# DichenZhang1/libultrahdr_dev

Hardware: AMD Instinct MI355X
Metric: MPixels/sec gain-map generate+apply, 4K P010 batch (higher is better)
Workload: dtype u8/u16 in, f32+f64 math, u8/u32 out

## Files before the change

libultrahdr_dev_amd/csrc/uhdr_capi.hip:

```cpp
#include <hip/hip_runtime.h>

#include <algorithm>
#include <memory>
#include <cmath>
#include <cstdio>
#include <cstring>
#include <map>
#include <chrono>
#include <mutex>
#include <thread>
#include <tuple>
#include <vector>

#include "../../include/uhdr_hip.h"
#include "uhdr_kernels.h"
#include "uhdr_jpeg.h"
#include "uhdr_jpegr.h"

namespace {

using namespace uhdr;

thread_local char t_err[256] = "";

void set_err(const char* where, hipError_t e) {
  snprintf(t_err, sizeof(t_err), "%s: %s", where, hipGetErrorString(e));
}

#define HIP_TRY(expr)                          \
  do {                                         \
    hipError_t _e = (expr);                    \
    if (_e != hipSuccess) {                    \
      set_err(#expr, _e);                      \
      return UHDR_HIP_UNKNOWN_ERROR;           \
    }                                          \
  } while (0)

constexpr int kStageSlots = 12;
struct StageSet {
  void* stage[kStageSlots] = {};
  size_t stage_bytes[kStageSlots] = {};
};
struct DeviceState : StageSet {
  bool ready = false;
  std::map<int, float*> idw;
  float* lut = nullptr;
  std::vector<std::unique_ptr<StageSet>> sets;
  std::vector<StageSet*> free_sets;
  std::vector<std::pair<hipStream_t, void*>> retired;
  std::vector<void*> pool;
  std::vector<size_t> pool_bytes;
  void* host_pool = nullptr;
  size_t host_pool_bytes = 0;
  std::map<hipStream_t, uint32_t*> stat_ws;
  struct ExWs { uint32_t* p = nullptr; size_t bytes = 0; };
  std::map<hipStream_t, ExWs> ex_ws;
  std::vector<std::unique_ptr<DeviceState>> codec_sets;
  std::vector<DeviceState*> free_codec;
};
std::mutex g_mu;
std::mutex g_pair_mu;
std::map<int, DeviceState> g_dev;

float euclid(float x1, float x2, float y1, float y2) {
  return (float)std::sqrt((double)(((y2 - y1) * (y2 - y1)) + (x2 - x1) * (x2 - x1)));
}
void fill_idw(float* w, int scale, int incR, int incB) {
  for (int y = 0; y < scale; y++)
    for (int x = 0; x < scale; x++) {
      const float pos_x = ((float)x) / scale, pos_y = ((float)y) / scale;
      const int curr_x = (int)std::floor((double)pos_x), curr_y = (int)std::floor((double)pos_y);
      const int next_x = curr_x + incR, next_y = curr_y + incB;
      const float d1 = euclid(pos_x, curr_x, pos_y, curr_y);
      float* o = w + y * scale * 4 + x * 4;
      if (d1 == 0) {
        o[0] = 1.f; o[1] = 0.f; o[2] = 0.f; o[3] = 0.f;
      } else {
        const float w1 = 1.f / d1;
        const float w2 = 1.f / euclid(pos_x, curr_x, pos_y, next_y);
        const float w3 = 1.f / euclid(pos_x, next_x, pos_y, curr_y);
        const float w4 = 1.f / euclid(pos_x, next_x, pos_y, next_y);
        const float total = w1 + w2 + w3 + w4;
        o[0] = w1 / total; o[1] = w2 / total; o[2] = w3 / total; o[3] = w4 / total;
      }
    }
}
void build_idw_tables(int scale, std::vector<float>& out) {
  const size_t n = (size_t)scale * scale * 4;
  out.assign(4 * n, 0.f);
  fill_idw(out.data(), scale, 1, 1);
  fill_idw(out.data() + n, scale, 0, 1);
  fill_idw(out.data() + 2 * n, scale, 1, 0);
  fill_idw(out.data() + 3 * n, scale, 0, 0);
}

int current_state(DeviceState** st) {
  int dev = -1;
  if (hipGetDevice(&dev) != hipSuccess) return UHDR_HIP_ERROR_INSUFFICIENT_RESOURCE;
  std::lock_guard<std::mutex> lk(g_mu);
  auto it = g_dev.find(dev);
  if (it == g_dev.end() || !it->second.ready) {
    snprintf(t_err, sizeof(t_err), "uhdr_hip_init(%d) has not been called", dev);
    return UHDR_HIP_ERROR_INSUFFICIENT_RESOURCE;
  }
  *st = &it->second;
  return UHDR_HIP_NO_ERROR;
}

constexpr int kIdwCacheMaxScale = 128;
int idw_for_scale(DeviceState* st, int scale, const float** dptr, float** transient) {
  *transient = nullptr;
  if (scale <= kIdwCacheMaxScale) {
    std::lock_guard<std::mutex> lk(g_mu);
    auto it = st->idw.find(scale);
    if (it != st->idw.end()) { *dptr = it->second; return UHDR_HIP_NO_ERROR; }
  }
  std::vector<float> t;
  try {
    build_idw_tables(scale, t);
  } catch (const std::bad_alloc&) {
    snprintf(t_err, sizeof(t_err), "no memory for the weight table of map scale %d", scale);
    return UHDR_HIP_ERROR_INSUFFICIENT_RESOURCE;
  }
  float* d = nullptr;
  if (hipMalloc(&d, t.size() * sizeof(float)) != hipSuccess) {
    (void)hipGetLastError();
    snprintf(t_err, sizeof(t_err), "no device memory for the weight table of map scale %d", scale);
    return UHDR_HIP_ERROR_INSUFFICIENT_RESOURCE;
  }
  if (hipMemcpy(d, t.data(), t.size() * sizeof(float), hipMemcpyHostToDevice) != hipSuccess) { (void)hipFree(d); return UHDR_HIP_UNKNOWN_ERROR; }
  if (scale > kIdwCacheMaxScale) { *transient = d; *dptr = d; return UHDR_HIP_NO_ERROR; }
  std::lock_guard<std::mutex> lk(g_mu);
  auto ins = st->idw.emplace(scale, d);
  if (!ins.second) (void)hipFree(d);
  *dptr = ins.first->second;
  return UHDR_HIP_NO_ERROR;
}

struct YuvRgb { float cr, gcb, gcr, cb; };
YuvRgb yuv_rgb_coeffs(int gamut) {
  switch (gamut) {
    case UHDR_HIP_CG_BT709: {
      const float R = 0.2126f, G = 0.7152f, B = 0.0722f, Cb = 1.8556f, Cr = 1.5748f;
      return {Cr, B * Cb / G, R * Cr / G, Cb};
    }
    case UHDR_HIP_CG_P3: {
      const float R = 0.299f, G = 0.587f, B = 0.114f, Cb = 1.772f, Cr = 1.402f;
      return {Cr, B * Cb / G, R * Cr / G, Cb};
    }
    default: {
      const float R = 0.2627f, G = 0.6780f, B = 0.0593f, Cb = 1.8814f, Cr = 1.4746f;
      return {Cr, B * Cb / G, R * Cr / G, Cb};
    }
  }
}
void luminance_coeffs(int gamut, float* o) {
  switch (gamut) {
    case UHDR_HIP_CG_BT709: o[0] = 0.2126f; o[1] = 0.7152f; o[2] = 0.0722f; break;
    case UHDR_HIP_CG_P3: o[0] = 0.20949f; o[1] = 0.72160f; o[2] = 0.06891f; break;
    default: o[0] = 0.2627f; o[1] = 0.6780f; o[2] = 0.0593f; break;
  }
}
const float kBt709ToP3[9] = {0.82254f, 0.17755f, 0.00006f, 0.03312f, 0.96684f, -0.00001f, 0.01706f, 0.07240f, 0.91049f};
const float kBt709ToBt2100[9] = {0.62740f, 0.32930f, 0.04332f, 0.06904f, 0.91958f, 0.01138f, 0.01636f, 0.08799f, 0.89555f};
const float kP3ToBt709[9] = {1.22482f, -0.22490f, -0.00007f, -0.04196f, 1.04199f, 0.00001f, -0.01961f, -0.07865f, 1.09831f};
const float kP3ToBt2100[9] = {0.75378f, 0.19862f, 0.04754f, 0.04576f, 0.94177f, 0.01250f, -0.00121f, 0.01757f, 0.98359f};
const float kBt2100ToBt709[9] = {1.66045f, -0.58764f, -0.07286f, -0.12445f, 1.13282f, -0.00837f, -0.01811f, -0.10057f, 1.11878f};
const float kBt2100ToP3[9] = {1.34369f, -0.28223f, -0.06135f, -0.06533f, 1.07580f, -0.01051f, 0.00283f, -0.01957f, 1.01679f};
const float* hdr_conversion(int sdr, int hdr) {
  if (sdr == hdr) return nullptr;
  switch (sdr) {
    case UHDR_HIP_CG_BT709: return hdr == UHDR_HIP_CG_P3 ? kP3ToBt709 : kBt2100ToBt709;
    case UHDR_HIP_CG_P3: return hdr == UHDR_HIP_CG_BT709 ? kBt709ToP3 : kBt2100ToP3;
    default: return hdr == UHDR_HIP_CG_BT709 ? kBt709ToBt2100 : kP3ToBt2100;
  }
}
const float kYuv709To601[9] = {1.0f, 0.101579f, 0.196076f, 0.0f, 0.989854f, -0.110653f, 0.0f, -0.072453f, 0.983398f};
const float kYuv709To2100[9] = {1.0f, -0.016969f, 0.096312f, 0.0f, 0.995306f, -0.051192f, 0.0f, 0.011507f, 1.002637f};
const float kYuv601To709[9] = {1.0f, -0.118188f, -0.212685f, 0.0f, 1.018640f, 0.114618f, 0.0f, 0.075049f, 1.025327f};
const float kYuv601To2100[9] = {1.0f, -0.128245f, -0.115879f, 0.0f, 1.010016f, 0.061592f, 0.0f, 0.086969f, 1.029350f};
const float kYuv2100To709[9] = {1.0f, 0.018149f, -0.095132f, 0.0f, 1.004123f, 0.051267f, 0.0f, -0.011524f, 0.996782f};
const float kYuv2100To601[9] = {1.0f, 0.117887f, 0.105521f, 0.0f, 0.995211f, -0.059549f, 0.0f, -0.084085f, 0.976518f};

bool valid_gamut(int g) { return g >= UHDR_HIP_CG_BT709 && g <= UHDR_HIP_CG_BT2100; }
bool al(const void* p, size_t a) { return (reinterpret_cast<uintptr_t>(p) % a) == 0; }

int validate_generate(const uhdr_hip_image_t* yuv, const uhdr_hip_image_t* p010, int hdr_tf,
                      const uhdr_hip_metadata_t* md, const uhdr_hip_image_t* dest) {
  if (yuv == nullptr || p010 == nullptr || md == nullptr || dest == nullptr || yuv->data == nullptr ||
      yuv->chroma_data == nullptr || p010->data == nullptr || p010->chroma_data == nullptr)
    return UHDR_HIP_ERROR_BAD_PTR;
  if (yuv->width != p010->width || yuv->height != p010->height) return UHDR_HIP_ERROR_RESOLUTION_MISMATCH;
  if (yuv->colorGamut == UHDR_HIP_CG_UNSPECIFIED || p010->colorGamut == UHDR_HIP_CG_UNSPECIFIED)
    return UHDR_HIP_ERROR_INVALID_COLORGAMUT;
  if (hdr_tf != UHDR_HIP_TF_LINEAR && hdr_tf != UHDR_HIP_TF_HLG && hdr_tf != UHDR_HIP_TF_PQ)
    return UHDR_HIP_ERROR_INVALID_TRANS_FUNC;
  if (!valid_gamut(yuv->colorGamut) || !valid_gamut(p010->colorGamut)) return UHDR_HIP_ERROR_INVALID_COLORGAMUT;
  return UHDR_HIP_NO_ERROR;
}

void fill_generate_metadata(int hdr_tf, uhdr_hip_metadata_t* md) {
  const float white = hdr_tf == UHDR_HIP_TF_PQ ? 10000.0f : 1000.0f;
  memset(md->version, 0, sizeof(md->version));
  strcpy(md->version, "1.0");
  md->maxContentBoost = white / 203.0f;
  md->minContentBoost = 1.0f;
  md->gamma = 1.0f;
  md->offsetSdr = 0.0f;
  md->offsetHdr = 0.0f;
  md->hdrCapacityMin = 1.0f;
  md->hdrCapacityMax = md->maxContentBoost;
}

void fill_generate_dest(const uhdr_hip_image_t* yuv, uhdr_hip_image_t* dest) {
  dest->width = yuv->width / 4;
  dest->height = yuv->height / 4;
  dest->colorGamut = UHDR_HIP_CG_UNSPECIFIED;
  dest->luma_stride = dest->width;
  dest->chroma_data = nullptr;
  dest->chroma_stride = 0;
  dest->pixelFormat = UHDR_HIP_PIX_FMT_MONOCHROME;
}

void encode_constants(float min_boost, float max_boost, float l2min, float l2max, double* scale, uint32_t* bmin,
                      uint32_t* bmax) {
  const double den = (double)(l2max - l2min);
  *scale = (double)255.0f / den;
  *bmin = (uint8_t)((std::log2((double)min_boost) - (double)l2min) / den * (double)255.0f);
  *bmax = (uint8_t)((std::log2((double)max_boost) - (double)l2min) / den * (double)255.0f);
}

GenConsts generate_consts(int sdr_gamut, int hdr_gamut, int hdr_tf, int sdr_is_601, size_t w, size_t h,
                          const uhdr_hip_metadata_t& md) {
  GenConsts c;
  const YuvRgb s = yuv_rgb_coeffs(sdr_is_601 ? UHDR_HIP_CG_P3 : sdr_gamut);
  const YuvRgb hh = yuv_rgb_coeffs(hdr_gamut);
  c.sdr_cr = s.cr; c.sdr_gcb = s.gcb; c.sdr_gcr = s.gcr; c.sdr_cb = s.cb;
  c.hdr_cr = hh.cr; c.hdr_gcb = hh.gcb; c.hdr_gcr = hh.gcr; c.hdr_cb = hh.cb;
  float l[3];
  luminance_coeffs(sdr_gamut, l);
  c.lum_r = l[0]; c.lum_g = l[1]; c.lum_b = l[2];
  const float* gm = hdr_conversion(sdr_gamut, hdr_gamut);
  c.gm_identity = gm == nullptr;
  for (int i = 0; i < 9; ++i) c.gm[i] = gm ? gm[i] : (i % 4 == 0 ? 1.0f : 0.0f);
  c.hdr_white_nits = hdr_tf == UHDR_HIP_TF_PQ ? 10000.0f : 1000.0f;
  c.min_boost = md.minContentBoost;
  c.max_boost = md.maxContentBoost;
  c.log2_min = (float)std::log2((double)md.minContentBoost);
  c.log2_max = (float)std::log2((double)md.maxContentBoost);
  encode_constants(c.min_boost, c.max_boost, c.log2_min, c.log2_max, &c.enc_scale, &c.enc_byte_min, &c.enc_byte_max);
  c.width = (uint32_t)w; c.height = (uint32_t)h;
  c.map_w = (uint32_t)(w / 4); c.map_h = (uint32_t)(h / 4);
  c.stat_keys = nullptr;
  c.stat_stride = 2;
  c.stat_ws = nullptr;
  c.stat_out = nullptr;
  c.stat_spread = 0u;
  c.stat_slots = 0u;
  c.lut = nullptr;
  c.bias4096 = 4096.0f;
  const double kRel = hdr_tf == UHDR_HIP_TF_PQ ? 1.0e-5 : 4.0e-6, kLogAbs = 5.0e-7;
  c.flt_scale = (float)c.enc_scale;
  c.flt_delta = (float)(1.25 * (c.enc_scale * (kRel * 1.4426950408889634 + kLogAbs) + 4.0e-5));
  c.flt_lo = (float)((double)c.min_boost * (1.0 - 2.0 * kRel));
  c.flt_hi = (float)((double)c.max_boost * (1.0 + 2.0 * kRel));
  c.flt_gain_rel = (float)(2.0 * kRel);
  return c;
}

GenImage gen_image(const uhdr_hip_image_t& yuv, const uhdr_hip_image_t& p010, void* map) {
  GenImage g;
  g.y = static_cast<const uint8_t*>(yuv.data);
  g.u = static_cast<const uint8_t*>(yuv.chroma_data);
  g.hy = static_cast<const uint16_t*>(p010.data);
  g.huv = static_cast<const uint16_t*>(p010.chroma_data);
  g.map = static_cast<uint8_t*>(map);
  g.y_stride = (uint32_t)yuv.luma_stride;
  g.c_stride = (uint32_t)yuv.chroma_stride;
  g.hy_stride = (uint32_t)(p010.luma_stride == 0 ? p010.width : p010.luma_stride);
  g.huv_stride = (uint32_t)p010.chroma_stride;
  return g;
}
bool gen_aligned(const GenImage& g, uint32_t w, uint32_t h) {
  const uint8_t* v = g.u + (size_t)g.c_stride * (h / 2u);
  if ((uint64_t)g.hy_stride * h >= (1ull << 31) || (uint64_t)g.y_stride * h >= (1ull << 32)) return false;
  return (w % 8u == 0) && al(g.hy, 16) && g.hy_stride % 8u == 0 && al(g.huv, 16) && g.huv_stride % 8u == 0 &&
         al(g.y, 8) && g.y_stride % 8u == 0 && al(g.u, 4) && al(v, 4) && g.c_stride % 4u == 0 && al(g.map, 2);
}

template <class F>
void chord(F f, double lo, double hi, double* c0, double* c1) {
  *c1 = (f(hi) - f(lo)) / (hi - lo);
  *c0 = f(lo) - *c1 * lo;
  double dev = 0.0;
  for (int k = 1; k < 32; ++k) { const double x = lo + (hi - lo) * k / 32.0; const double d = f(x) - (*c0 + *c1 * x); if (std::fabs(d) > std::fabs(dev)) dev = d; }
  *c0 += 0.5 * dev;
}
void f16_cell(uint32_t j, double* lo, double* hi) {
  const uint32_t e = j >> 7, m = j & 127u;
  if (e == 0) { *lo = std::ldexp((double)m, -21); *hi = std::ldexp((double)(m + 1u), -21); return; }
  *lo = std::ldexp(1.0 + m / 128.0, (int)e - 15);
  *hi = std::ldexp(1.0 + (m + 1u) / 128.0, (int)e - 15);
}
void f32_cell16(uint32_t j, double* lo, double* hi) {
  const uint32_t e = 96u + (j >> 4), m = j & 15u;
  *lo = std::ldexp(1.0 + m / 16.0, (int)e - 127);
  *hi = std::ldexp(1.0 + (m + 1u) / 16.0, (int)e - 127);
}
void build_stage1(double g, float* out) {
  const double thr = (double)0.04045f;
  auto eotf = [&](double x) { return x <= thr ? x / (double)12.92f : std::pow((x + (double)0.055f) / (double)1.055f, 2.4); };
  auto f = [&](double x) { return g == 1.0 ? eotf(x) : std::pow(eotf(x), g); };
  const uint32_t cells = (g == 1.0 ? kTabS1Bytes : kTabS1PowBytes) / 8u;
  for (uint32_t j = 0; j < cells; ++j) {
    double lo, hi, c0, c1;
    if (g == 1.0) f16_cell(j, &lo, &hi); else f32_cell16(j, &lo, &hi);
    if (g == 1.0 && hi <= thr) { c0 = 0.0; c1 = 1.0 / (double)12.92f; }
    else if (lo >= 1.0) { c0 = 1.0; c1 = 0.0; }
    else if (j == 0) { c0 = 0.0; c1 = f(hi) / hi; }
    else chord(f, lo, hi, &c0, &c1);
    out[2 * j] = (float)c0; out[2 * j + 1] = (float)c1;
  }
}
template <class F>
void build_stage2(F code_of_u, float* out) {
  for (uint32_t k = 0; k < kTabS2Cells; ++k) {
    const double lo = 2.0 + k / 64.0, hi = 2.0 + (k + 1u) / 64.0;
    auto f = [&](double s) { return code_of_u(std::min(1.0, 0.5 * (s - 2.0))); };
    float c0f = -2.0f, c1f = 0.0f;
    if (k == kTabS2Cells - 1u) c0f = (float)(-2.0 - std::ldexp(1023.0, -22));
    else if (f(hi) >= 0.99) {
      double c0, c1;
      chord(f, lo, hi, &c0, &c1);
      c0 += 1.0 / 256.0;
      const double n = c0 < 0.0 ? std::nearbyint(2.0 * c0) / 2.0 : std::nearbyint(c0);
      c1 += (c0 - n) / (0.5 * (lo + hi));
      c0f = (float)(-2.0 - std::ldexp(n, -22));
      c1f = (float)(-std::ldexp(c1, -22));
      auto at = [&](double s) { return -(((double)c1f * s + (double)c0f) + 2.0) * 4194304.0; };
      for (int it = 0; it < 4096 && at(lo) < 0.0; ++it) c1f = std::nextafter(c1f, -INFINITY);
      if (at(lo) < 0.0) { c0f = -2.0f; c1f = 0.0f; }
    }
    out[2 * k] = c0f; out[2 * k + 1] = c1f;
  }
}
void build_line_tables(std::vector<float>& tab) {
  tab.assign(kTabEnd - kTabS1Lin, 0.0f);
  const double m1 = (double)(2610.0f / 16384.0f), m2 = (double)(2523.0f / 4096.0f * 128.0f);
  const double k1 = (double)(3424.0f / 4096.0f), k2 = (double)(2413.0f / 4096.0f * 32.0f), k3 = (double)(2392.0f / 4096.0f * 32.0f);
  build_stage1(1.0, tab.data() + (kTabS1Lin - kTabS1Lin));
  build_stage1(0.5, tab.data() + (kTabS1Hlg - kTabS1Lin));
  build_stage1(m1, tab.data() + (kTabS1Pq - kTabS1Lin));
  auto hlg = [](double u) { const double x = u * u; return 1023.0 * (x <= 1.0 / 12.0 ? std::sqrt(3.0) * u : (double)0.17883277f * std::log(12.0 * x - (double)0.28466892f) + (double)0.55991073f); };
  auto pq = [&](double p) { return p <= 0.0 ? 0.0 : 1023.0 * std::pow((k1 + k2 * p) / (1.0 + k3 * p), m2); };
  build_stage2(hlg, tab.data() + (kTabS2Hlg - kTabS1Lin));
  build_stage2(pq, tab.data() + (kTabS2Pq - kTabS1Lin));
}

int validate_apply(const uhdr_hip_image_t* yuv, const uhdr_hip_image_t* map, const uhdr_hip_metadata_t* md,
                   const uhdr_hip_image_t* dest) {
  if (yuv == nullptr || map == nullptr || md == nullptr || dest == nullptr || yuv->data == nullptr ||
      yuv->chroma_data == nullptr || map->data == nullptr)
    return UHDR_HIP_ERROR_BAD_PTR;
  if (strncmp(md->version, "1.0", sizeof(md->version)) != 0) return UHDR_HIP_ERROR_BAD_METADATA;
  if (md->gamma != 1.0f) return UHDR_HIP_ERROR_BAD_METADATA;
  if (md->offsetSdr != 0.0f || md->offsetHdr != 0.0f) return UHDR_HIP_ERROR_BAD_METADATA;
  if (md->hdrCapacityMin != md->minContentBoost || md->hdrCapacityMax != md->maxContentBoost)
    return UHDR_HIP_ERROR_BAD_METADATA;
  if (map->width == 0 || map->height == 0) return UHDR_HIP_ERROR_UNSUPPORTED_MAP_SCALE_FACTOR;
  if (yuv->width % map->width != 0 || yuv->height % map->height != 0)
    return UHDR_HIP_ERROR_UNSUPPORTED_MAP_SCALE_FACTOR;
  if (yuv->width * map->height != yuv->height * map->width) return UHDR_HIP_ERROR_UNSUPPORTED_MAP_SCALE_FACTOR;
  return UHDR_HIP_NO_ERROR;
}
bool apply_writes(int fmt) {
  return fmt == UHDR_HIP_OUTPUT_HDR_LINEAR || fmt == UHDR_HIP_OUTPUT_HDR_PQ || fmt == UHDR_HIP_OUTPUT_HDR_HLG ||
         fmt == UHDR_HIP_OUTPUT_HDR_LINEAR_RGB_10BIT;
}
size_t apply_bpp(int fmt) {
  return fmt == UHDR_HIP_OUTPUT_HDR_LINEAR ? 8 : fmt == UHDR_HIP_OUTPUT_HDR_LINEAR_RGB_10BIT ? 6 : 4;
}
AppConsts apply_consts(const uhdr_hip_image_t& yuv, const uhdr_hip_image_t& map, const uhdr_hip_metadata_t& md,
                       float max_display_boost, const float* idw) {
  AppConsts c;
  c.width = (uint32_t)yuv.width; c.height = (uint32_t)yuv.height;
  c.map_w = (uint32_t)map.width; c.map_h = (uint32_t)map.height;
  c.scale = (uint32_t)(yuv.width / map.width);
  c.display_boost = (std::min)(max_display_boost, md.maxContentBoost);
  c.inv_display_boost = 1.0f / c.display_boost;
  c.max_boost = md.maxContentBoost;
  c.inv_max_boost = 1.0f / md.maxContentBoost;
  c.log2_min_d = std::log2((double)md.minContentBoost);
  c.log2_max_d = std::log2((double)md.maxContentBoost);
  c.idw = idw;
  c.lut = nullptr;
  c.lut_boost_factor = c.display_boost > 0 ? c.display_boost / md.maxContentBoost : 1.0f;
  const double lut_top = std::exp2(std::fmax(c.log2_min_d, c.log2_max_d) * (double)c.lut_boost_factor) / (double)c.display_boost;
  c.lut_plain_div = (c.display_boost >= 0x1p-20f && c.display_boost <= 0x1p20f && std::fabs(c.log2_min_d * (double)c.lut_boost_factor) <= 40.0 &&
                     std::fabs(c.log2_max_d * (double)c.lut_boost_factor) <= 40.0 && lut_top <= 32768.0) ? 1u : 0u;
  const double ratio = (double)c.display_boost / (double)md.maxContentBoost;
  c.fast.A = (float)((c.log2_max_d - c.log2_min_d) * ratio);
  c.fast.B = (float)(c.log2_min_d * ratio - std::log2((double)c.display_boost));
  c.fast.A255 = (float)((c.log2_max_d - c.log2_min_d) * ratio / 255.0);
  std::vector<float> t;
  build_idw_tables(4, t);
  for (int oy = 0; oy < 4; ++oy)
    for (int pr = 0; pr < 2; ++pr)
      for (int k = 1; k < 4; ++k)
        for (int j = 0; j < 2; ++j)
          c.fast.wD[oy][pr][k - 1][j] = t[oy * 16 + (2 * pr + j) * 4 + k];
  c.tab = nullptr;
  c.ex_ws = nullptr;
  c.ex_cap = 0;
  c.cells_per_thread = 8;
  c.step_x = c.step_y = 0;
  return c;
}
AppImage app_image(const uhdr_hip_image_t& yuv, const uhdr_hip_image_t& map, void* dst) {
  AppImage a;
  a.y = static_cast<const uint8_t*>(yuv.data);
  a.u = static_cast<const uint8_t*>(yuv.chroma_data);
  a.v = a.u + yuv.chroma_stride * (yuv.height / 2);
  a.map = static_cast<const uint8_t*>(map.data);
  a.dst = dst;
  a.y_stride = (uint32_t)yuv.luma_stride;
  a.c_stride = (uint32_t)yuv.chroma_stride;
  return a;
}
bool app_fast_s4(const AppConsts& c, const AppImage& a) {
  if ((uint64_t)a.y_stride * c.height >= (1ull << 32) || (uint64_t)c.width * c.height >= (1ull << 29)) return false;
  return c.scale == 4 && c.width == 4u * c.map_w && c.height == 4u * c.map_h && al(a.y, 4) && a.y_stride % 4u == 0 &&
         al(a.u, 2) && al(a.v, 2) && a.c_stride % 2u == 0 && al(a.dst, 16);
}
void fill_apply_dest(const uhdr_hip_image_t* yuv, uhdr_hip_image_t* dest) {
  dest->width = yuv->width;
  dest->height = yuv->height;
  dest->colorGamut = yuv->colorGamut;
}

int stage_reserve(StageSet* st, int slot, size_t bytes) {
  if (bytes == 0) bytes = 256;
  if (st->stage_bytes[slot] >= bytes) return UHDR_HIP_NO_ERROR;
  if (st->stage[slot]) HIP_TRY(hipFree(st->stage[slot]));
  st->stage[slot] = nullptr;
  st->stage_bytes[slot] = 0;
  HIP_TRY(hipMalloc(&st->stage[slot], bytes));
  st->stage_bytes[slot] = bytes;
  return UHDR_HIP_NO_ERROR;
}
size_t round_up(size_t v, size_t a) { return (v + a - 1) / a * a; }

class StageLease {
 public:
  explicit StageLease(DeviceState* st) : st_(st) {
    std::lock_guard<std::mutex> lk(g_mu);
    if (st_->free_sets.empty()) {
      try {
        st_->sets.emplace_back(new StageSet());
        set_ = st_->sets.back().get();
      } catch (const std::bad_alloc&) {
        set_ = nullptr;
      }
    } else {
      set_ = st_->free_sets.back();
      st_->free_sets.pop_back();
    }
  }
  ~StageLease() {
    if (set_ == nullptr) return;
    std::lock_guard<std::mutex> lk(g_mu);
    try { st_->free_sets.push_back(set_); } catch (const std::bad_alloc&) {}
  }
  StageLease(const StageLease&) = delete;
  StageLease& operator=(const StageLease&) = delete;
  StageSet* get() const { return set_; }
 private:
  DeviceState* st_;
  StageSet* set_;
};

class CodecLease {
 public:
  explicit CodecLease(DeviceState* st) : st_(st) {
    std::lock_guard<std::mutex> lk(g_mu);
    if (!st_->free_codec.empty()) {
      ctx_ = st_->free_codec.back();
      st_->free_codec.pop_back();
    } else {
      try {
        st_->free_codec.reserve(st_->codec_sets.size() + 1);
        st_->codec_sets.emplace_back(new DeviceState());
        ctx_ = st_->codec_sets.back().get();
      } catch (const std::bad_alloc&) {
        ctx_ = nullptr;
      }
    }
    if (ctx_) { ctx_->ready = true; ctx_->lut = st_->lut; }
  }
  ~CodecLease() {
    if (ctx_ == nullptr) return;
    std::lock_guard<std::mutex> lk(g_mu);
    st_->free_codec.push_back(ctx_);
  }
  CodecLease(const CodecLease&) = delete;
  CodecLease& operator=(const CodecLease&) = delete;
  DeviceState* get() const { return ctx_; }

 private:
  DeviceState* st_;
  DeviceState* ctx_ = nullptr;
};

int h2d_plane(void* d, size_t dpitch_elems, const void* h, size_t hstride_elems, size_t row_elems, size_t rows,
              size_t esz, hipStream_t s) {
  if (rows == 0 || row_elems == 0) return UHDR_HIP_NO_ERROR;
  if (hstride_elems == 0) {
    for (size_t r = 0; r < rows; ++r)
      HIP_TRY(hipMemcpyAsync(static_cast<char*>(d) + r * dpitch_elems * esz, h, row_elems * esz, hipMemcpyHostToDevice, s));
    return UHDR_HIP_NO_ERROR;
  }
  HIP_TRY(hipMemcpy2DAsync(d, dpitch_elems * esz, h, hstride_elems * esz, row_elems * esz, rows, hipMemcpyHostToDevice, s));
  return UHDR_HIP_NO_ERROR;
}
int d2h_plane(void* h, size_t hstride_elems, const void* d, size_t dpitch_elems, size_t row_elems, size_t rows,
              size_t esz, hipStream_t s) {
  if (rows == 0 || row_elems == 0) return UHDR_HIP_NO_ERROR;
  HIP_TRY(hipMemcpy2DAsync(h, hstride_elems * esz, d, dpitch_elems * esz, row_elems * esz, rows, hipMemcpyDeviceToHost, s));
  return UHDR_HIP_NO_ERROR;
}

int stage_yuv420_in(StageSet* st, int slot, const uhdr_hip_image_t& h, uhdr_hip_image_t* d, hipStream_t s) {
  const size_t w = h.width, hh = h.height, cw = (w + 1) / 2, ch = (hh + 1) / 2;
  const size_t lp = round_up(w ? w : 1, 64), cp = round_up(cw ? cw : 1, 64);
  int rc;
  if ((rc = stage_reserve(st, slot, lp * (hh ? hh : 1))) != 0) return rc;
  if ((rc = stage_reserve(st, slot + 1, cp * ((hh / 2) + ch + 1))) != 0) return rc;
  *d = h;
  d->data = st->stage[slot];
  d->chroma_data = st->stage[slot + 1];
  d->luma_stride = lp;
  d->chroma_stride = cp;
  if ((rc = h2d_plane(d->data, lp, h.data, h.luma_stride, w, hh, 1, s)) != 0) return rc;
  const uint8_t* hu = static_cast<const uint8_t*>(h.chroma_data);
  const uint8_t* hv = hu + h.chroma_stride * (hh / 2);
  uint8_t* du = static_cast<uint8_t*>(d->chroma_data);
  if ((rc = h2d_plane(du, cp, hu, h.chroma_stride, cw, ch, 1, s)) != 0) return rc;
  if ((rc = h2d_plane(du + cp * (hh / 2), cp, hv, h.chroma_stride, cw, ch, 1, s)) != 0) return rc;
  return UHDR_HIP_NO_ERROR;
}
int stage_p010_in(StageSet* st, int slot, const uhdr_hip_image_t& h, uhdr_hip_image_t* d, hipStream_t s) {
  const size_t w = h.width, hh = h.height, cw2 = ((w + 1) / 2) * 2, ch = (hh + 1) / 2;
  const size_t lp = round_up(w ? w : 1, 64), cp = round_up(cw2 ? cw2 : 2, 64);
  int rc;
  if ((rc = stage_reserve(st, slot, lp * (hh ? hh : 1) * 2)) != 0) return rc;
  if ((rc = stage_reserve(st, slot + 1, cp * (ch ? ch : 1) * 2)) != 0) return rc;
  *d = h;
  d->data = st->stage[slot];
  d->chroma_data = st->stage[slot + 1];
  d->luma_stride = lp;
  d->chroma_stride = cp;
  const size_t hls = h.luma_stride == 0 ? h.width : h.luma_stride;
// ... 1897 lines not shown
    memset(&e.sdr, 0, sizeof(e.sdr));
    if (api3) {
      const uint8_t* ip = nullptr;
      size_t in = 0;
      e.sdr_gamut = jpegr::first_icc(static_cast<const uint8_t*>(sdr_jpeg[i]), sdr_jpeg_size[i], &ip, &in) ? jpegr::gamut_from_icc(ip, in) : sdr_jpeg_gamut[i];
    } else {
      e.sdr = yuv420_images[i];
      default_yuv(&e.sdr);
      e.sdr_gamut = e.sdr.colorGamut;
      e.icc = std::move(icc[i]);
    }
    files.push_back(std::move(e));
  }
  auto result = [&]() {
    int first = UHDR_HIP_NO_ERROR;
    for (int i = 0; i < n; ++i) { if (status) status[i] = st_[i]; if (first == UHDR_HIP_NO_ERROR) first = st_[i]; }
    return first;
  };
  if (files.empty()) return result();
  DeviceState* st = nullptr;
  int rc = current_state(&st);
  size_t r0 = 0;
  if (rc == UHDR_HIP_NO_ERROR) {
    CodecLease lease(st);
    st = lease.get();
    rc = st == nullptr ? UHDR_HIP_ERROR_INSUFFICIENT_RESOURCE : UHDR_HIP_NO_ERROR;
    hipStream_t s = static_cast<hipStream_t>(stream);
    const bool host = mem_space != UHDR_HIP_MEM_DEVICE;
    auto key = [](const SjFile& e) { return std::make_tuple(e.p010.width, e.p010.height, e.sdr_gamut, e.p010.colorGamut); };
    std::stable_sort(files.begin(), files.end(), [&](const SjFile& x, const SjFile& y) { return key(x) < key(y); });
    struct SyncOnExit {
      hipStream_t s;
      ~SyncOnExit() { (void)hipStreamSynchronize(s); }
    } sync_on_exit{s};
    while (rc == UHDR_HIP_NO_ERROR && r0 < files.size()) {
      size_t r1 = r0, bytes = 0;
      while (r1 < files.size() && r1 - r0 < (size_t)kEncRound) {
        const size_t b = sj_round_bytes(files[r1], api3 ? &info[files[r1].idx] : nullptr, host);
        if (r1 > r0 && bytes + b > kCodecRoundBytes) break;
        bytes += b;
        ++r1;
      }
      rc = sdr_jpeg_round(st, s, api3, host, hdr_tf, &files[r0], (int)(r1 - r0), sdr_jpeg, sdr_jpeg_size, sdr_jpeg_gamut, api3 ? info.data() : nullptr,
                          dec_out.data(), dec_need.data(), out, out_capacity, out_size, st_.data());
      if (rc == UHDR_HIP_NO_ERROR) r0 = r1;
    }
  }
  for (size_t k = r0; k < files.size(); ++k)
    if (st_[files[k].idx] == UHDR_HIP_NO_ERROR) st_[files[k].idx] = rc;
  return result();
}

struct XFile {
  int idx = 0;
  uhdr_hip_image_t yuv, map;
  std::vector<uint8_t> icc;
};

int apix_round(DeviceState* st, hipStream_t s, bool host, int quality, const XFile* f, int m, const uhdr_hip_metadata_t* metadata,
               const void* const* exif, const size_t* exif_size, void* const* out, const size_t* out_capacity, size_t* out_size, int* st_) {
  std::vector<EncJpeg> jpg;
  jpg.reserve(2 * (size_t)m);
  int rc;
  if (host) {
    size_t total = 0;
    for (int k = 0; k < m; ++k) total += enc_stage_bytes(f[k].yuv) + enc_stage_bytes(f[k].map);
    if ((rc = pool_reserve(st, kEncYuv, total)) != 0) return rc;
  }
  size_t o = 0;
  for (int k = 0; k < m; ++k) {
    const XFile& e = f[k];
    jpg.push_back(EncJpeg{e.yuv, quality, &e.icc, e.yuv.luma_stride, e.yuv.chroma_stride});
    jpg.push_back(gainmap_jpeg(e.map, e.map.luma_stride));
    if (!host) continue;
    uint8_t* pool = static_cast<uint8_t*>(st->pool[kEncYuv]);
    if ((rc = stage_encoder_slice(pool + o, e.yuv, &jpg[2 * (size_t)k].img, s)) != 0) return rc;
    o += enc_stage_bytes(e.yuv);
    if ((rc = stage_encoder_slice(pool + o, e.map, &jpg[2 * (size_t)k + 1].img, s)) != 0) return rc;
    o += enc_stage_bytes(e.map);
  }
  if (compress_to_host(st, s, 2 * m, jpg.data()) != UHDR_HIP_NO_ERROR) return UHDR_HIP_ERROR_ENCODE_ERROR;
  on_host_threads(m, [&](int lo, int hi) {
    for (int k = lo; k < hi; ++k) {
      const int i = f[k].idx;
      const EncJpeg& sdr = jpg[2 * (size_t)k];
      const EncJpeg& gm = jpg[2 * (size_t)k + 1];
      st_[i] = jpegr::append_gainmap_to(sdr.bytes, sdr.n, gm.bytes, gm.n, static_cast<const uint8_t*>(exif ? exif[i] : nullptr), exif ? exif_size[i] : 0,
                                        nullptr, 0, metadata[i], static_cast<uint8_t*>(out[i]), out_capacity[i], &out_size[i]);
    }
  });
  return UHDR_HIP_NO_ERROR;
}
}

extern "C" {

int uhdr_hip_jpegr_encode_sdr_jpeg_batch(int n, const uhdr_hip_image_t* p010_images, const uhdr_hip_image_t* yuv420_images,
                                         const void* const* sdr_jpeg, const size_t* sdr_jpeg_size, const int* sdr_jpeg_gamut, int hdr_tf,
                                         void* const* out, const size_t* out_capacity, size_t* out_size, int* status, int mem_space, void* stream) {
  if (n < 0 || (n > 0 && (p010_images == nullptr || sdr_jpeg == nullptr || sdr_jpeg_size == nullptr || sdr_jpeg_gamut == nullptr || out == nullptr ||
                          out_capacity == nullptr || out_size == nullptr)))
    return UHDR_HIP_ERROR_BAD_PTR;
  return sdr_jpeg_files(n, p010_images, yuv420_images, sdr_jpeg, sdr_jpeg_size, sdr_jpeg_gamut, hdr_tf, out, out_capacity, out_size, status,
                        mem_space, stream);
}

int uhdr_hip_jpegr_encode_apix_batch(int n, const uhdr_hip_image_t* yuv420_images, const uhdr_hip_image_t* gainmap_images,
                                     const uhdr_hip_metadata_t* metadata, int quality, const void* const* exif, const size_t* exif_size,
                                     void* const* out, const size_t* out_capacity, size_t* out_size, int* status, int mem_space, void* stream) {
  if (n < 0 || (n > 0 && (yuv420_images == nullptr || gainmap_images == nullptr || metadata == nullptr || out == nullptr || out_capacity == nullptr ||
                          out_size == nullptr)) ||
      (exif != nullptr && exif_size == nullptr))
    return UHDR_HIP_ERROR_BAD_PTR;
  if (quality < 0 || quality > 100) return UHDR_HIP_ERROR_INVALID_QUALITY_FACTOR;
  std::vector<int> st_((size_t)n, UHDR_HIP_NO_ERROR);
  std::vector<XFile> files;
  for (int i = 0; i < n; ++i) {
    const uhdr_hip_image_t& y = yuv420_images[i];
    const uhdr_hip_image_t& g = gainmap_images[i];
    if (y.data == nullptr || g.data == nullptr || out[i] == nullptr) { st_[i] = UHDR_HIP_ERROR_BAD_PTR; continue; }
    XFile e;
    e.idx = i;
    int rc = apix_check(y, g, &e.yuv, &e.map, &e.icc);
    if (rc == UHDR_HIP_NO_ERROR && !jpegr::metadata_valid(metadata[i])) rc = UHDR_HIP_ERROR_BAD_METADATA;
    if (rc != UHDR_HIP_NO_ERROR) { st_[i] = rc; continue; }
    files.push_back(std::move(e));
  }
  auto result = [&]() {
    int first = UHDR_HIP_NO_ERROR;
    for (int i = 0; i < n; ++i) { if (status) status[i] = st_[i]; if (first == UHDR_HIP_NO_ERROR) first = st_[i]; }
    return first;
  };
  if (files.empty()) return result();
  DeviceState* st = nullptr;
  int rc = current_state(&st);
  size_t r0 = 0;
  if (rc == UHDR_HIP_NO_ERROR) {
    CodecLease lease(st);
    st = lease.get();
    rc = st == nullptr ? UHDR_HIP_ERROR_INSUFFICIENT_RESOURCE : UHDR_HIP_NO_ERROR;
    hipStream_t s = static_cast<hipStream_t>(stream);
    const bool host = mem_space != UHDR_HIP_MEM_DEVICE;
    struct SyncOnExit {
      hipStream_t s;
      ~SyncOnExit() { (void)hipStreamSynchronize(s); }
    } sync_on_exit{s};
    while (rc == UHDR_HIP_NO_ERROR && r0 < files.size()) {
      size_t r1 = r0, bytes = 0;
      while (r1 < files.size() && r1 - r0 < (size_t)kEncRound) {
        const size_t b = enc_round_bytes(files[r1].yuv, host, true) + enc_round_bytes(files[r1].map, host, true);
        if (r1 > r0 && bytes + b > kCodecRoundBytes) break;
        bytes += b;
        ++r1;
      }
      rc = apix_round(st, s, host, quality, &files[r0], (int)(r1 - r0), metadata, exif, exif_size, out, out_capacity, out_size, st_.data());
      if (rc == UHDR_HIP_NO_ERROR) r0 = r1;
    }
  }
  for (size_t k = r0; k < files.size(); ++k) st_[files[k].idx] = rc;
  return result();
}

int uhdr_hip_jpegr_info(const void* jpegr, size_t jpegr_size, uhdr_hip_jpeg_info_t* primary, uhdr_hip_jpeg_info_t* gainmap) {
  if (jpegr == nullptr || primary == nullptr) return UHDR_HIP_ERROR_BAD_PTR;
  const uint8_t* file = static_cast<const uint8_t*>(jpegr);
  jpegr::Range img[2];
  const int found = jpegr::find_images(file, jpegr_size, img);
  if (found == 0) return UHDR_HIP_ERROR_NO_IMAGES_FOUND;
  if (found == 1) return UHDR_HIP_ERROR_GAIN_MAP_IMAGE_NOT_FOUND;
  auto parse = [&](const jpegr::Range& r, uhdr_hip_jpeg_info_t* info) -> int {
    const uint8_t* j = file + r.begin;
    struct { int w, h; } di;
    if (!jpegr::has_valid_header(j, r.len) || !jpegr::dimensions(j, r.len, &di.w, &di.h)) return UHDR_HIP_ERROR_DECODE_ERROR;
    if (di.w > 8192 || di.h > 8192) return UHDR_HIP_ERROR_DECODE_ERROR;
    memset(info, 0, sizeof(*info));
    info->offset = r.begin; info->size = r.len;
    info->width = (size_t)di.w; info->height = (size_t)di.h;
    jpegr::first_packets(j, r.len, &info->xmp_offset, &info->xmp_size, &info->exif_offset, &info->exif_size, &info->icc_offset, &info->icc_size);
    if (info->xmp_size) info->xmp_offset += r.begin;
    if (info->exif_size) info->exif_offset += r.begin;
    if (info->icc_size) info->icc_offset += r.begin;
    return UHDR_HIP_NO_ERROR;
  };
  int rc = parse(img[0], primary);
  if (rc != UHDR_HIP_NO_ERROR) return rc;
  return gainmap != nullptr ? parse(img[1], gainmap) : UHDR_HIP_NO_ERROR;
}

int uhdr_hip_jpegr_metadata(const void* jpegr, size_t jpegr_size, uhdr_hip_metadata_t* metadata) {
  if (jpegr == nullptr || metadata == nullptr) return UHDR_HIP_ERROR_BAD_PTR;
  const uint8_t* file = static_cast<const uint8_t*>(jpegr);
  jpegr::Range img[2];
  const int found = jpegr::find_images(file, jpegr_size, img);
  if (found == 0) return UHDR_HIP_ERROR_NO_IMAGES_FOUND;
  if (found == 1) return UHDR_HIP_ERROR_GAIN_MAP_IMAGE_NOT_FOUND;
  const uint8_t* xmp = nullptr;
  size_t xmp_len = 0;
  if (!jpegr::first_xmp(file + img[1].begin, img[1].len, &xmp, &xmp_len) ||
      !jpegr::metadata_from_xmp(xmp, xmp_len, metadata))
    return UHDR_HIP_ERROR_METADATA_ERROR;
  return UHDR_HIP_NO_ERROR;
}

int uhdr_hip_lut_table(int which, float* out, size_t capacity, size_t* count) {
  if (out == nullptr || count == nullptr) return UHDR_HIP_ERROR_BAD_PTR;
  DeviceState* st = nullptr;
  const int rc = current_state(&st);
  if (rc != UHDR_HIP_NO_ERROR) return rc;
  uint32_t off = 0, n = 0;
  switch (which) {
    case 0: off = kLutSrgbInv; n = kLutSrgbInvN; break;
    case 1: off = kLutHlgInv; n = kLutHlgInvN; break;
    case 2: off = kLutPqInv; n = kLutPqInvN; break;
    case 4: off = kLutHlg; n = kLutHlgN; break;
    case 5: off = kLutPq; n = kLutPqN; break;
    default: return UHDR_HIP_ERROR_UNSUPPORTED_FEATURE;
  }
  *count = n;
  if (capacity < n) return UHDR_HIP_ERROR_INSUFFICIENT_RESOURCE;
  HIP_TRY(hipMemcpy(out, st->lut + off, sizeof(float) * n, hipMemcpyDeviceToHost));
  return UHDR_HIP_NO_ERROR;
}

int uhdr_hip_gain_lut(const uhdr_hip_metadata_t* metadata, int with_display_boost, float display_boost, float* out) {
  if (metadata == nullptr || out == nullptr) return UHDR_HIP_ERROR_BAD_PTR;
  DeviceState* st = nullptr;
  int rc = current_state(&st);
  if (rc != UHDR_HIP_NO_ERROR) return rc;
  float factor = 1.0f;
  if (with_display_boost) factor = display_boost > 0 ? display_boost / metadata->maxContentBoost : 1.0f;
  CodecLease lease(st);
  if ((st = lease.get()) == nullptr) return UHDR_HIP_ERROR_INSUFFICIENT_RESOURCE;
  if ((rc = stage_reserve(st, 6, sizeof(float) * kGainLutN)) != 0) return rc;
  float* d = static_cast<float*>(st->stage[6]);
  HIP_TRY(launch_build_gain_lut(d, std::log2((double)metadata->minContentBoost), std::log2((double)metadata->maxContentBoost),
                                factor, nullptr));
  HIP_TRY(hipMemcpy(out, d, sizeof(float) * kGainLutN, hipMemcpyDeviceToHost));
  return UHDR_HIP_NO_ERROR;
}

int uhdr_hip_idw_tables(int scale, float* out) {
  if (out == nullptr || scale <= 0) return UHDR_HIP_ERROR_BAD_PTR;
  std::vector<float> t;
  build_idw_tables(scale, t);
  memcpy(out, t.data(), t.size() * sizeof(float));
  return UHDR_HIP_NO_ERROR;
}

int uhdr_hip_generate_gainmap_batch(int n, const uhdr_hip_image_t* yuvs, const uhdr_hip_image_t* p010s, int hdr_tf,
                                    uhdr_hip_metadata_t* metadata, uhdr_hip_image_t* dests, int sdr_is_601,
                                    float* content_minmax, void* stream) {
  return uhdr_hip_generate_gainmap_batch_ex(n, yuvs, p010s, hdr_tf, metadata, dests, sdr_is_601, UHDR_HIP_GENERATE_EXACT,
                                            content_minmax, stream);
}

int uhdr_hip_generate_gainmap_batch_ex(int n, const uhdr_hip_image_t* yuvs, const uhdr_hip_image_t* p010s, int hdr_tf,
                                       uhdr_hip_metadata_t* metadata, uhdr_hip_image_t* dests, int sdr_is_601,
                                       int generate_mode, float* content_minmax, void* stream) {
  if (generate_mode != UHDR_HIP_GENERATE_EXACT && generate_mode != UHDR_HIP_GENERATE_LUT &&
      generate_mode != UHDR_HIP_GENERATE_UNFILTERED)
    return UHDR_HIP_ERROR_UNSUPPORTED_FEATURE;
  const bool lut = generate_mode == UHDR_HIP_GENERATE_LUT;
  if (n < 0 || (n > 0 && (yuvs == nullptr || p010s == nullptr || dests == nullptr)) || metadata == nullptr)
    return UHDR_HIP_ERROR_BAD_PTR;
  for (int i = 0; i < n; ++i) {
    const int rc = validate_generate(&yuvs[i], &p010s[i], hdr_tf, metadata, &dests[i]);
    if (rc != UHDR_HIP_NO_ERROR) return rc;
    if (dests[i].data == nullptr) return UHDR_HIP_ERROR_BAD_PTR;
  }
  if (hdr_tf != UHDR_HIP_TF_LINEAR && hdr_tf != UHDR_HIP_TF_HLG && hdr_tf != UHDR_HIP_TF_PQ)
    return UHDR_HIP_ERROR_INVALID_TRANS_FUNC;
  DeviceState* st = nullptr;
  int rc = current_state(&st);
  if (rc != UHDR_HIP_NO_ERROR) return rc;
  hipStream_t s = static_cast<hipStream_t>(stream);

  fill_generate_metadata(hdr_tf, metadata);
  uint32_t* keys = reinterpret_cast<uint32_t*>(content_minmax);

  int i = 0;
  while (i < n) {
    const uhdr_hip_image_t& y0 = yuvs[i];
    GenConsts c = generate_consts(y0.colorGamut, p010s[i].colorGamut, hdr_tf, sdr_is_601, y0.width, y0.height, *metadata);
    c.stat_keys = keys ? keys + 2 * i : nullptr;
    c.stat_stride = 2;
    c.lut = lut ? st->lut : nullptr;
    GenBatch b;
    int m = 0;
    bool aligned = true;
    while (i + m < n && m < kMaxChunk) {
      const uhdr_hip_image_t& y = yuvs[i + m];
      if (y.width != y0.width || y.height != y0.height || y.colorGamut != y0.colorGamut ||
          p010s[i + m].colorGamut != p010s[i].colorGamut)
        break;
      b.img[m] = gen_image(y, p010s[i + m], dests[i + m].data);
      const bool a = gen_aligned(b.img[m], c.width, c.height);
      if (m == 0) aligned = a;
      else if (a != aligned) break;
      fill_generate_dest(&y, &dests[i + m]);
      ++m;
    }
    bool filter = generate_mode == UHDR_HIP_GENERATE_EXACT && c.flt_delta < 0.25f && c.min_boost >= 0.25f && c.max_boost <= 64.0f;
    const bool small = generate_is_small(c, m);
    const bool pair = keys != nullptr ? generate_resolve_pays(c, m) : !small;
    if (keys != nullptr && !pair) filter = false;
    const bool resolve = filter && aligned && !lut && pair;
    std::unique_lock<std::mutex> pair_lk(g_pair_mu, std::defer_lock);
    if (resolve) pair_lk.lock();
    if (resolve) {
      uint32_t* w = nullptr;
      const int wrc = stat_workspace(st, s, &w);
      if (wrc != UHDR_HIP_NO_ERROR) return wrc;
      c.stat_ws = w;
      c.stat_keys = keys ? w + 4 : nullptr;
      c.stat_stride = kStatWords;
      c.stat_out = keys ? content_minmax + 2 * i : nullptr;
      c.stat_spread = (m <= 16 && (uint64_t)((c.map_w + 1u) >> 1) * c.map_h >= 512u * 64u) ? 1u : 0u;
      c.stat_slots = generate_slot_waves(c, m);
    } else if (keys != nullptr) {
      HIP_TRY(launch_stats_init(keys + 2 * i, m, s));
    }
    HIP_TRY(launch_generate(c, b, m, hdr_tf, aligned, lut, filter, s));
    if (resolve) HIP_TRY(launch_stats_resolve(c, b, m, hdr_tf, aligned, s));
    else if (keys != nullptr) HIP_TRY(launch_stats_finalize(keys + 2 * i, m, s));
    i += m;
  }
  return UHDR_HIP_NO_ERROR;
}

int uhdr_hip_apply_gainmap_batch(int n, const uhdr_hip_image_t* yuvs, const uhdr_hip_image_t* maps,
                                 const uhdr_hip_metadata_t* metadata, int output_format, float max_display_boost,
                                 uhdr_hip_image_t* dests, int apply_mode, void* stream) {
  if (n < 0 || (n > 0 && (yuvs == nullptr || maps == nullptr || dests == nullptr)) || metadata == nullptr)
    return UHDR_HIP_ERROR_BAD_PTR;
  for (int i = 0; i < n; ++i) {
    const int rc = validate_apply(&yuvs[i], &maps[i], metadata, &dests[i]);
    if (rc != UHDR_HIP_NO_ERROR) return rc;
  }
  if (apply_mode != UHDR_HIP_APPLY_FAST && apply_mode != UHDR_HIP_APPLY_EXACT && apply_mode != UHDR_HIP_APPLY_LUT &&
      apply_mode != UHDR_HIP_APPLY_EXACT_UNFILTERED)
    return UHDR_HIP_ERROR_UNSUPPORTED_FEATURE;
  DeviceState* st = nullptr;
  int rc = current_state(&st);
  if (rc != UHDR_HIP_NO_ERROR) return rc;
  hipStream_t s = static_cast<hipStream_t>(stream);
  const bool writes = apply_writes(output_format);
  for (int i = 0; i < n; ++i)
    if (writes && dests[i].data == nullptr) return UHDR_HIP_ERROR_BAD_PTR;

  int i = 0;
  while (i < n) {
    const uhdr_hip_image_t& y0 = yuvs[i];
    const uhdr_hip_image_t& m0 = maps[i];
    const int scale = (int)(y0.width / m0.width);
    const float* idw = nullptr;
    float* idw_transient = nullptr;
    if ((rc = idw_for_scale(st, scale, &idw, &idw_transient)) != UHDR_HIP_NO_ERROR) return rc;
    struct FreeAfter {
      float* p; hipStream_t s;
      ~FreeAfter() { if (p) { (void)hipStreamSynchronize(s); (void)hipFree(p); } }
    } free_after{idw_transient, s};
    AppConsts c = apply_consts(y0, m0, *metadata, max_display_boost, idw);
    c.lut = apply_mode == UHDR_HIP_APPLY_LUT ? st->lut : nullptr;
    c.tab = st->lut;
    AppBatch b;
    int m = 0;
    bool fast = true;
    while (i + m < n && m < kMaxChunk) {
      const uhdr_hip_image_t& y = yuvs[i + m];
      const uhdr_hip_image_t& mp = maps[i + m];
      if (y.width != y0.width || y.height != y0.height || mp.width != m0.width || mp.height != m0.height) break;
      b.img[m] = app_image(y, mp, dests[i + m].data);
      const bool f = app_fast_s4(c, b.img[m]);
      if (m == 0) fast = f;
      else if (f != fast) break;
      fill_apply_dest(&y, &dests[i + m]);
      ++m;
    }
    std::unique_lock<std::mutex> pair_lk(g_pair_mu, std::defer_lock);
    if (writes && apply_mode == UHDR_HIP_APPLY_EXACT && (uint64_t)c.width * c.height <= 0xFFFFFFFFull &&
        std::fabs(c.log2_min_d) <= 32.0 && std::fabs(c.log2_max_d) <= 32.0) {
      pair_lk.lock();
      const uint32_t cap = ex_list_cap((uint64_t)c.width * c.height);
      uint32_t* w = nullptr;
      const int wrc = exact_workspace(st, s, m, cap, &w);
      if (wrc != UHDR_HIP_NO_ERROR) return wrc;
      c.ex_ws = w;
      c.ex_cap = cap;
    }
    if (writes) HIP_TRY(launch_apply(c, b, m, output_format, apply_mode, fast, s));
    i += m;
  }
  return UHDR_HIP_NO_ERROR;
}

int uhdr_hip_generate_gainmap(const uhdr_hip_image_t* yuv, const uhdr_hip_image_t* p010, int hdr_tf,
                              uhdr_hip_metadata_t* metadata, uhdr_hip_image_t* dest, int sdr_is_601, int mem_space,
                              void* stream) {
  return uhdr_hip_generate_gainmap_ex(yuv, p010, hdr_tf, metadata, dest, sdr_is_601, UHDR_HIP_GENERATE_EXACT, mem_space, stream);
}

int uhdr_hip_generate_gainmap_ex(const uhdr_hip_image_t* yuv, const uhdr_hip_image_t* p010, int hdr_tf,
                                 uhdr_hip_metadata_t* metadata, uhdr_hip_image_t* dest, int sdr_is_601, int generate_mode,
                                 int mem_space, void* stream) {
  int rc = validate_generate(yuv, p010, hdr_tf, metadata, dest);
  if (rc != UHDR_HIP_NO_ERROR) return rc;
  if (dest->data == nullptr) return UHDR_HIP_ERROR_BAD_PTR;
  if (mem_space == UHDR_HIP_MEM_DEVICE)
    return uhdr_hip_generate_gainmap_batch_ex(1, yuv, p010, hdr_tf, metadata, dest, sdr_is_601, generate_mode, nullptr, stream);

  DeviceState* st = nullptr;
  if ((rc = current_state(&st)) != UHDR_HIP_NO_ERROR) return rc;
  StageLease lease(st);
  StageSet* ss = lease.get();
  if (ss == nullptr) return UHDR_HIP_ERROR_INSUFFICIENT_RESOURCE;
  hipStream_t s = static_cast<hipStream_t>(stream);
  uhdr_hip_image_t dy, dp, dm = *dest;
  if ((rc = stage_yuv420_in(ss, 0, *yuv, &dy, s)) != 0) return rc;
  if ((rc = stage_p010_in(ss, 2, *p010, &dp, s)) != 0) return rc;
  const size_t mw = yuv->width / 4, mh = yuv->height / 4;
  if ((rc = stage_reserve(ss, 4, mw * mh)) != 0) return rc;
  dm.data = ss->stage[4];
  rc = uhdr_hip_generate_gainmap_batch_ex(1, &dy, &dp, hdr_tf, metadata, &dm, sdr_is_601, generate_mode, nullptr, stream);
  if (rc != UHDR_HIP_NO_ERROR) return rc;
  if (mw * mh) HIP_TRY(hipMemcpyAsync(dest->data, dm.data, mw * mh, hipMemcpyDeviceToHost, s));
  HIP_TRY(hipStreamSynchronize(s));
  fill_generate_dest(yuv, dest);
  return UHDR_HIP_NO_ERROR;
}

int uhdr_hip_apply_gainmap(const uhdr_hip_image_t* yuv, const uhdr_hip_image_t* map, const uhdr_hip_metadata_t* metadata,
                           int output_format, float max_display_boost, uhdr_hip_image_t* dest, int apply_mode,
                           int mem_space, void* stream) {
  int rc = validate_apply(yuv, map, metadata, dest);
  if (rc != UHDR_HIP_NO_ERROR) return rc;
  if (mem_space == UHDR_HIP_MEM_DEVICE)
    return uhdr_hip_apply_gainmap_batch(1, yuv, map, metadata, output_format, max_display_boost, dest, apply_mode, stream);

  const bool writes = apply_writes(output_format);
  if (writes && dest->data == nullptr) return UHDR_HIP_ERROR_BAD_PTR;
  DeviceState* st = nullptr;
  if ((rc = current_state(&st)) != UHDR_HIP_NO_ERROR) return rc;
  StageLease lease(st);
  StageSet* ss = lease.get();
  if (ss == nullptr) return UHDR_HIP_ERROR_INSUFFICIENT_RESOURCE;
  hipStream_t s = static_cast<hipStream_t>(stream);
  uhdr_hip_image_t dy, dm = *map, dd = *dest;
  if ((rc = stage_yuv420_in(ss, 0, *yuv, &dy, s)) != 0) return rc;
  const size_t map_bytes = map->width * map->height;
  if ((rc = stage_reserve(ss, 4, map_bytes)) != 0) return rc;
  HIP_TRY(hipMemcpyAsync(ss->stage[4], map->data, map_bytes, hipMemcpyHostToDevice, s));
  dm.data = ss->stage[4];
  const size_t out_bytes = writes ? yuv->width * yuv->height * apply_bpp(output_format) : 0;
  if ((rc = stage_reserve(ss, 5, out_bytes)) != 0) return rc;
  dd.data = ss->stage[5];
  rc = uhdr_hip_apply_gainmap_batch(1, &dy, &dm, metadata, output_format, max_display_boost, &dd, apply_mode, stream);
  if (rc != UHDR_HIP_NO_ERROR) return rc;
  if (out_bytes) HIP_TRY(hipMemcpyAsync(dest->data, dd.data, out_bytes, hipMemcpyDeviceToHost, s));
  HIP_TRY(hipStreamSynchronize(s));
  fill_apply_dest(yuv, dest);
  return UHDR_HIP_NO_ERROR;
}

namespace {
ToneImage tone_image(const uhdr_hip_image_t& sd, const uhdr_hip_image_t& dd, bool* aligned) {
  ToneImage t;
  t.sy = static_cast<const uint16_t*>(sd.data);
  t.suv = static_cast<const uint16_t*>(sd.chroma_data);
  t.dy = static_cast<uint8_t*>(dd.data);
  t.du = static_cast<uint8_t*>(dd.chroma_data);
  t.dv = t.du + (dd.chroma_stride * dd.height / 2);
  t.sy_stride = (uint32_t)sd.luma_stride; t.suv_stride = (uint32_t)sd.chroma_stride;
  t.dy_stride = (uint32_t)dd.luma_stride; t.dc_stride = (uint32_t)dd.chroma_stride;
  t.width = (uint32_t)sd.width; t.height = (uint32_t)sd.height;
  *aligned = t.width % 16u == 0 && al(t.sy, 16) && t.sy_stride % 8u == 0 && al(t.suv, 16) &&
             t.suv_stride % 8u == 0 && al(t.dy, 8) && t.dy_stride % 8u == 0 && t.dy_stride >= t.width &&
             al(t.du, 8) && al(t.dv, 8) && t.dc_stride % 8u == 0 && t.dc_stride >= t.width / 2u;
  return t;
}
int tonemap_check(const uhdr_hip_image_t* src, const uhdr_hip_image_t* dest) {
  if (src == nullptr || dest == nullptr) return UHDR_HIP_ERROR_BAD_PTR;
  if (src->width != dest->width || src->height != dest->height) return UHDR_HIP_ERROR_RESOLUTION_MISMATCH;
  if (src->data == nullptr || src->chroma_data == nullptr || dest->data == nullptr || dest->chroma_data == nullptr)
    return UHDR_HIP_ERROR_BAD_PTR;
  return UHDR_HIP_NO_ERROR;
}
}

int uhdr_hip_tonemap_batch(int n, const uhdr_hip_image_t* srcs, uhdr_hip_image_t* dests, void* stream) {
  if (n < 0 || (n > 0 && (srcs == nullptr || dests == nullptr))) return UHDR_HIP_ERROR_BAD_PTR;
  for (int i = 0; i < n; ++i) {
    const int rc = tonemap_check(&srcs[i], &dests[i]);
    if (rc != UHDR_HIP_NO_ERROR) return rc;
  }
  DeviceState* st = nullptr;
  int rc = current_state(&st);
  if (rc != UHDR_HIP_NO_ERROR) return rc;
  hipStream_t s = static_cast<hipStream_t>(stream);
  int i = 0;
  while (i < n) {
    ToneBatch b;
    bool aligned = true;
    int m = 0;
    while (i + m < n && m < kToneChunk) {
      bool a;
      const ToneImage t = tone_image(srcs[i + m], dests[i + m], &a);
      if (m == 0) aligned = a;
      else if (a != aligned || t.width != b.img[0].width || t.height != b.img[0].height) break;
      b.img[m++] = t;
    }
    HIP_TRY(launch_tonemap(b, m, aligned, s));
    for (int k = 0; k < m; ++k) dests[i + k].colorGamut = srcs[i + k].colorGamut;
    i += m;
  }
  return UHDR_HIP_NO_ERROR;
}

int uhdr_hip_tonemap(const uhdr_hip_image_t* src, uhdr_hip_image_t* dest, int mem_space, void* stream) {
  int rc = tonemap_check(src, dest);
  if (rc != UHDR_HIP_NO_ERROR) return rc;
  if (mem_space == UHDR_HIP_MEM_DEVICE) return uhdr_hip_tonemap_batch(1, src, dest, stream);
  DeviceState* st = nullptr;
  if ((rc = current_state(&st)) != UHDR_HIP_NO_ERROR) return rc;
  hipStream_t s = static_cast<hipStream_t>(stream);

  auto run = [&](const uhdr_hip_image_t& sd, const uhdr_hip_image_t& dd) -> int {
    ToneBatch b;
    bool aligned;
    b.img[0] = tone_image(sd, dd, &aligned);
    HIP_TRY(launch_tonemap(b, 1, aligned, s));
    return UHDR_HIP_NO_ERROR;
  };

  StageLease lease(st);
  StageSet* ss = lease.get();
  if (ss == nullptr) return UHDR_HIP_ERROR_INSUFFICIENT_RESOURCE;
  uhdr_hip_image_t ds, dd = *dest;
  if ((rc = stage_p010_in(ss, 2, *src, &ds, s)) != 0) return rc;
  const size_t h = dest->height, ls = dest->luma_stride, cs = dest->chroma_stride;
  if ((rc = stage_reserve(ss, 0, ls * h)) != 0) return rc;
  if ((rc = stage_reserve(ss, 1, cs * h + cs)) != 0) return rc;
  dd.data = ss->stage[0];
  dd.chroma_data = ss->stage[1];
  if ((rc = run(ds, dd)) != 0) return rc;
  if (ls * h) HIP_TRY(hipMemcpyAsync(dest->data, dd.data, ls * h, hipMemcpyDeviceToHost, s));
  const size_t v_off = cs * h / 2;
  if (cs * (h / 2)) {
    HIP_TRY(hipMemcpyAsync(dest->chroma_data, dd.chroma_data, cs * (h / 2), hipMemcpyDeviceToHost, s));
    HIP_TRY(hipMemcpyAsync(static_cast<uint8_t*>(dest->chroma_data) + v_off, static_cast<uint8_t*>(dd.chroma_data) + v_off,
                           cs * (h / 2), hipMemcpyDeviceToHost, s));
  }
  HIP_TRY(hipStreamSynchronize(s));
  dest->colorGamut = src->colorGamut;
  return UHDR_HIP_NO_ERROR;
}

namespace {
int convert_check(const uhdr_hip_image_t* image, int src_encoding, int dest_encoding) {
  if (image == nullptr) return UHDR_HIP_ERROR_BAD_PTR;
  if (src_encoding == UHDR_HIP_CG_UNSPECIFIED || dest_encoding == UHDR_HIP_CG_UNSPECIFIED)
    return UHDR_HIP_ERROR_INVALID_COLORGAMUT;
  if (!valid_gamut(src_encoding) || !valid_gamut(dest_encoding)) return UHDR_HIP_ERROR_INVALID_COLORGAMUT;
  return UHDR_HIP_NO_ERROR;
}
}

int uhdr_hip_convert_yuv_batch(int n, uhdr_hip_image_t* images, int src_encoding, int dest_encoding, void* stream) {
  if (n < 0 || (n > 0 && images == nullptr)) return UHDR_HIP_ERROR_BAD_PTR;
  int rc = convert_check(n > 0 ? &images[0] : nullptr, src_encoding, dest_encoding);
  if (n == 0) rc = (src_encoding == UHDR_HIP_CG_UNSPECIFIED || dest_encoding == UHDR_HIP_CG_UNSPECIFIED || !valid_gamut(src_encoding) ||
                    !valid_gamut(dest_encoding)) ? UHDR_HIP_ERROR_INVALID_COLORGAMUT : UHDR_HIP_NO_ERROR;
  if (rc != UHDR_HIP_NO_ERROR) return rc;
  if (src_encoding == dest_encoding) return UHDR_HIP_NO_ERROR;
  for (int i = 0; i < n; ++i)
    if (images[i].data == nullptr || images[i].chroma_data == nullptr) return UHDR_HIP_ERROR_BAD_PTR;
  const float* m = yuv_matrix(src_encoding, dest_encoding);
  DeviceState* st = nullptr;
  if ((rc = current_state(&st)) != UHDR_HIP_NO_ERROR) return rc;
  hipStream_t s = static_cast<hipStream_t>(stream);
  int i = 0;
  while (i < n) {
    CvtBatch b;
    bool aligned = true;
    int k = 0;
    while (i + k < n && k < kToneChunk) {
      bool a;
      const CvtImage t = cvt_image(images[i + k], images[i + k], m, &a);
      if (k == 0) aligned = a;
      else if (a != aligned || t.width != b.img[0].width || t.height != b.img[0].height) break;
      b.img[k++] = t;
    }
    HIP_TRY(launch_convert_yuv(b, k, aligned, s));
    i += k;
  }
  return UHDR_HIP_NO_ERROR;
}

int uhdr_hip_convert_yuv(uhdr_hip_image_t* image, int src_encoding, int dest_encoding, int mem_space, void* stream) {
  int rc = convert_check(image, src_encoding, dest_encoding);
  if (rc != UHDR_HIP_NO_ERROR) return rc;
  if (src_encoding == dest_encoding) return UHDR_HIP_NO_ERROR;
  if (image->data == nullptr || image->chroma_data == nullptr) return UHDR_HIP_ERROR_BAD_PTR;
  if (mem_space == UHDR_HIP_MEM_DEVICE) return uhdr_hip_convert_yuv_batch(1, image, src_encoding, dest_encoding, stream);
  const float* m = yuv_matrix(src_encoding, dest_encoding);
  DeviceState* st = nullptr;
  if ((rc = current_state(&st)) != UHDR_HIP_NO_ERROR) return rc;
  hipStream_t s = static_cast<hipStream_t>(stream);
  auto run = [&](const uhdr_hip_image_t& d) -> int { return convert_yuv_into(d, d, m, s); };
  StageLease lease(st);
  if (lease.get() == nullptr) return UHDR_HIP_ERROR_INSUFFICIENT_RESOURCE;
  uhdr_hip_image_t d;
  if ((rc = stage_yuv420_in(lease.get(), 0, *image, &d, s)) != 0) return rc;
  if ((rc = run(d)) != 0) return rc;
  const size_t w = image->width, h = image->height, cw = w / 2, ch = h / 2;
  if ((rc = d2h_plane(image->data, image->luma_stride, d.data, d.luma_stride, cw * 2, ch * 2, 1, s)) != 0) return rc;
  uint8_t* hu = static_cast<uint8_t*>(image->chroma_data);
  const uint8_t* du = static_cast<const uint8_t*>(d.chroma_data);
  if ((rc = d2h_plane(hu, image->chroma_stride, du, d.chroma_stride, cw, ch, 1, s)) != 0) return rc;
  if ((rc = d2h_plane(hu + image->chroma_stride * (h / 2), image->chroma_stride, du + d.chroma_stride * (h / 2),
                      d.chroma_stride, cw, ch, 1, s)) != 0)
    return rc;
  HIP_TRY(hipStreamSynchronize(s));
  return UHDR_HIP_NO_ERROR;
}

namespace {
enum { FXK_CROP, FXK_MIRROR, FXK_ROTATE, FXK_RESIZE };
// ... 227 lines not shown
```

libultrahdr_dev_amd/csrc/uhdr_kernels.h:

```cpp
#pragma once
#include <hip/hip_runtime_api.h>
#include <stdint.h>

namespace uhdr {

constexpr uint32_t kStatSlotWaves = 1024, kStatSlotPlain = 15, kStatSlotSaved = 4, kStatSlotWords = 16 + 16 * kStatSlotSaved;
constexpr uint32_t kStatLists = 64, kStatCap = 252, kStatEst = 8 + kStatLists, kStatSlotCnt = kStatEst + 2 * kStatLists,
                   kStatHdr = kStatSlotCnt + kStatSlotWaves,
                   kStatWords = kStatHdr + (kStatLists * kStatCap > kStatSlotWaves * kStatSlotWords ? kStatLists * kStatCap : kStatSlotWaves * kStatSlotWords);
static_assert(kStatHdr % 4u == 0u && kStatSlotWords % 4u == 0u && kStatWords % 4u == 0u, "saved entries are read and written as 16-byte pieces");
constexpr int kMaxChunk = 64;

constexpr uint32_t kLutSrgbInvN = 1024, kLutHlgInvN = 4096, kLutPqInvN = 4096, kLutHlgN = 65536, kLutPqN = 65536;
constexpr uint32_t kLutSrgbInv = 0, kLutHlgInv = kLutSrgbInv + kLutSrgbInvN, kLutPqInv = kLutHlgInv + kLutHlgInvN,
                   kLutHlg = kLutPqInv + kLutPqInvN, kLutPq = kLutHlg + kLutHlgN, kLutTotal = kLutPq + kLutPqN;
constexpr uint32_t kTabS1Bytes = 0x3C00 + 16;
constexpr uint32_t kTabS1PowBytes = 512u * 8u;
constexpr uint32_t kTabS2Cells = 129, kTabS2Floats = 260;
constexpr uint32_t kTabS2LdsBytes = kTabS2Cells * 256u;
constexpr uint32_t kTabS1Lin = kLutTotal, kTabS1Hlg = kTabS1Lin + kTabS1Bytes / 4, kTabS1Pq = kTabS1Hlg + kTabS1PowBytes / 4,
                   kTabS2Hlg = kTabS1Pq + kTabS1PowBytes / 4, kTabS2Pq = kTabS2Hlg + kTabS2Floats, kTabEnd = kTabS2Pq + kTabS2Floats;
constexpr uint32_t kCodeHlg = kTabEnd, kCodePq = kCodeHlg + kLutHlgN / 2, kLutBufferFloats = kCodePq + kLutPqN / 2;
constexpr uint32_t kGainLutN = 1024;

struct GenConsts {
  float sdr_cr, sdr_gcb, sdr_gcr, sdr_cb;
  float hdr_cr, hdr_gcb, hdr_gcr, hdr_cb;
  float lum_r, lum_g, lum_b;
  float gm[9];
  int gm_identity;
  float hdr_white_nits;
  float bias4096;
  float min_boost, max_boost, log2_min, log2_max;
  double enc_scale;
  uint32_t enc_byte_min, enc_byte_max;
  uint32_t width, height, map_w, map_h;
  uint32_t* stat_keys;
  uint32_t stat_stride;
  uint32_t* stat_ws;
  float* stat_out;
  const float* lut;
  float flt_scale, flt_delta, flt_lo, flt_hi;
  float flt_gain_rel;
  uint32_t stat_spread;
  uint32_t stat_slots;
};
struct EvalConsts {
  float min_boost, max_boost, log2_min, log2_max;
  double enc_scale;
  uint32_t enc_byte_min, enc_byte_max;
  const float* lut;
  double log2_min_d, log2_max_d;
};
struct GenImage {
  const uint8_t* y;
  const uint8_t* u;
  const uint16_t* hy;
  const uint16_t* huv;
  uint8_t* map;
  uint32_t y_stride, c_stride, hy_stride, huv_stride;
};
struct GenBatch {
  GenImage img[kMaxChunk];
};

struct AppFast {
  float A, B, A255;
  float wD[4][2][3][2];
};
struct AppConsts {
  uint32_t width, height, map_w, map_h, scale;
  uint32_t cells_per_thread;
  uint32_t step_x, step_y;
  float display_boost, inv_display_boost, max_boost, inv_max_boost;
  double log2_min_d, log2_max_d;
  const float* idw;
  const float* lut;
  const float* tab;
  float lut_boost_factor;
  uint32_t lut_plain_div;
  uint32_t* ex_ws;
  uint32_t ex_cap;
  AppFast fast;
};
constexpr uint32_t kExLists = 1024;
constexpr uint32_t kExHdrWords = 8 + kExLists;
inline size_t ex_ws_bytes(uint32_t cap) { return ((size_t)kMaxChunk * kExHdrWords + (size_t)kMaxChunk * kExLists * cap) * 4u; }
inline uint32_t ex_list_cap(uint64_t pixels) { return (uint32_t)(pixels / 16u / kExLists) + 64u; }
struct AppImage {
  const uint8_t* y;
  const uint8_t* u;
  const uint8_t* v;
  const uint8_t* map;
  void* dst;
  uint32_t y_stride, c_stride;
};
struct AppBatch {
  AppImage img[kMaxChunk];
};

struct ToneImage {
  const uint16_t* sy;
  const uint16_t* suv;
  uint8_t* dy;
  uint8_t* du;
  uint8_t* dv;
  uint32_t sy_stride, suv_stride, dy_stride, dc_stride;
  uint32_t width, height;
};
constexpr int kToneChunk = 32;
struct ToneBatch {
  ToneImage img[kToneChunk];
};
struct CvtImage {
  uint8_t* y;
  uint8_t* u;
  uint8_t* v;
  uint32_t y_stride, c_stride, width, height;
  float m[9];
  const uint8_t* sy;
  const uint8_t* su;
  const uint8_t* sv;
  uint32_t sy_stride, sc_stride;
};
struct CvtBatch {
  CvtImage img[kToneChunk];
};

enum FxOp : int { FX_COPY = 0, FX_FLIP_V, FX_FLIP_H, FX_ROT90, FX_ROT180, FX_ROT270, FX_RESIZE };
struct FxJob {
  const uint8_t* src;
  uint8_t* dst;
  uint32_t rows, cols, dst_stride, src_stride;
  uint32_t in_w, in_h;
  uint32_t row_num, row_den, col_num, col_den;
  int op;
};
struct FxJobs {
  FxJob job[3];
  int n;
};

static_assert(sizeof(GenConsts) + sizeof(GenBatch) <= 4096, "generate kernel arguments exceed the kernarg segment");
static_assert(sizeof(AppConsts) + sizeof(AppBatch) <= 4096, "apply kernel arguments exceed the kernarg segment");

hipError_t launch_generate(const GenConsts& c, const GenBatch& b, int n, int hdr_tf, bool aligned, bool lut,
                           bool filter, hipStream_t s);
bool generate_is_small(const GenConsts& c, int n);
bool generate_resolve_pays(const GenConsts& c, int n);
uint32_t generate_slot_waves(const GenConsts& c, int n);
hipError_t launch_stats_init(uint32_t* keys, int n, hipStream_t s);
hipError_t launch_stats_resolve(const GenConsts& c, const GenBatch& b, int n, int hdr_tf, bool aligned, hipStream_t s);
constexpr size_t kStatWsBytes = sizeof(uint32_t) * kStatWords * (size_t)kMaxChunk;
hipError_t launch_stats_finalize(uint32_t* keys, int n, hipStream_t s);
hipError_t launch_apply(const AppConsts& c, const AppBatch& b, int n, int fmt, int mode,
                        bool fast_s4, hipStream_t s);
hipError_t launch_build_luts(float* lut , hipStream_t s);
hipError_t launch_build_lut_codes(float* lut , hipStream_t s);
hipError_t launch_build_gain_lut(float* table, double log2_min, double log2_max, float boost_factor, hipStream_t s);
hipError_t launch_tonemap(const ToneBatch& b, int n, bool aligned, hipStream_t s);
hipError_t launch_convert_yuv(const CvtBatch& b, int n, bool aligned, hipStream_t s);
static_assert(sizeof(CvtBatch) <= 4096 && sizeof(ToneBatch) <= 4096, "toneMap / convertYuv kernel arguments exceed the kernarg segment");
hipError_t launch_ycc420_to_rgba(const uint8_t* y, const uint8_t* cb, const uint8_t* cr, uint32_t w, uint32_t h, uint32_t y_stride,
                                 uint32_t c_stride, uint8_t* rgba, hipStream_t s);
constexpr int kRgbaChunk = 64;
struct YccRgbaImage {
  const uint8_t* y;
  const uint8_t* cb;
  const uint8_t* cr;
  uint8_t* rgba;
  uint32_t w, h, ys, cs;
};
struct YccRgbaBatch {
  YccRgbaImage img[kRgbaChunk];
};
static_assert(sizeof(YccRgbaBatch) <= 4096, "k_ycc420_rgba_batch's kernel arguments exceed the kernarg segment");
hipError_t launch_ycc420_to_rgba_batch(const YccRgbaBatch& b, int n, hipStream_t s);
hipError_t upload_idw4(const float* tables );
hipError_t launch_effect(const FxJobs& j, hipStream_t s);
hipError_t launch_eval_transfer(int fn, const float* in, float* out, size_t n, const EvalConsts& ec, hipStream_t s);
hipError_t launch_synth_lcg(uint16_t* p010, uint8_t* yuv, uint32_t n_luma, uint32_t n, uint32_t seed, hipStream_t s);

}
```

libultrahdr_dev_amd/csrc/uhdr_kernels.hip:

```cpp
#include "uhdr_kernels.h"

#include <hip/hip_runtime.h>

#include <algorithm>
#include <cmath>

#include "uhdr_device_math.h"
#include "uhdr_wave_scan.h"

namespace uhdr {

__constant__ float c_idw4[4 * 64];

__constant__ float c_idw4p[64];

hipError_t upload_idw4(const float* tables) {
  float p[64];
  for (int oy = 0; oy < 4; ++oy)
    for (int pr = 0; pr < 2; ++pr)
      for (int k = 0; k < 4; ++k)
        for (int h = 0; h < 2; ++h) p[((oy * 2 + pr) * 4 + k) * 2 + h] = tables[oy * 16 + (2 * pr + h) * 4 + k];
  hipError_t e = hipMemcpyToSymbol(HIP_SYMBOL(c_idw4p), p, sizeof(p));
  if (e != hipSuccess) return e;
  return hipMemcpyToSymbol(HIP_SYMBOL(c_idw4), tables, sizeof(float) * 4 * 64);
}

constexpr float k255 = 1 / 255.0f;
constexpr float k876 = 1 / 876.0f;
constexpr float k896 = 1 / 896.0f;

constexpr float kP3YR = 0.299f, kP3YG = 0.587f, kP3YB = 0.114f;
constexpr float kP3Cb = 1.772f, kP3Cr = 1.402f;
constexpr float kP3GCb = kP3YB * kP3Cb / kP3YG;
constexpr float kP3GCr = kP3YR * kP3Cr / kP3YG;

typedef float f2 __attribute__((ext_vector_type(2)));
__device__ __forceinline__ f2 pk_fma(f2 a, f2 b, f2 c) { return __builtin_elementwise_fma(a, b, c); }
__device__ __forceinline__ f2 splat(float v) { return (f2){v, v}; }
__device__ __forceinline__ f2 bc_lo(f2 v) { return __builtin_shufflevector(v, v, 0, 0); }
__device__ __forceinline__ f2 bc_hi(f2 v) { return __builtin_shufflevector(v, v, 1, 1); }

__device__ __forceinline__ f2 pk_add_sat(f2 a, f2 b) {
  f2 r;
  asm("v_pk_add_f32 %0, %1, %2 clamp" : "=v"(r) : "v"(a), "v"(b));
  return r;
}
__device__ __forceinline__ f2 pk_mul_sat(f2 a, f2 b) {
  f2 r;
  asm("v_pk_mul_f32 %0, %1, %2 clamp" : "=v"(r) : "v"(a), "v"(b));
  return r;
}
__device__ __forceinline__ f2 pk_fma_sat(f2 a, f2 b, f2 c) {
  f2 r;
  asm("v_pk_fma_f32 %0, %1, %2, %3 clamp" : "=v"(r) : "v"(a), "v"(b), "v"(c));
  return r;
}

template <int HI>
__device__ __forceinline__ f2 pk_fma_sat_bc(f2 a, f2 b, f2 c) {
  f2 r;
  if (HI) asm("v_pk_fma_f32 %0, %1, %2, %3 op_sel:[0,0,1] op_sel_hi:[1,1,1] clamp" : "=v"(r) : "v"(a), "v"(b), "v"(c));
  else asm("v_pk_fma_f32 %0, %1, %2, %3 op_sel_hi:[1,1,0] clamp" : "=v"(r) : "v"(a), "v"(b), "v"(c));
  return r;
}


__device__ __attribute__((noinline)) uint32_t lut_index_wild(float t) {
  const double pos = (double)t + 0.5;
  uint32_t v = 0u;
  if (__builtin_fabs(pos) < 9223372036854775808.0) v = (uint32_t)(long long)pos;
  return v;
}
__device__ __forceinline__ uint32_t round_half_up(float t) {
  int r;
  asm("v_cvt_rpi_i32_f32 %0, %1" : "=v"(r) : "v"(t));
  return (uint32_t)r;
}
__device__ __forceinline__ uint32_t lut_index(float e, uint32_t n) {
  const float t = e * (float)(n - 1u);
  uint32_t v;
  if (__builtin_expect(__float_as_uint(t) < 0x4F000000u, 1)) v = round_half_up(t);
  else v = lut_index_wild(t);
  return min(v, n - 1u);
}
__device__ __forceinline__ uint32_t lut_index_unit(float e, uint32_t n) {
  return round_half_up(e * (float)(n - 1u));
}
__device__ __forceinline__ float gain_lut_entry(uint32_t idx, double log2_min, double log2_max, float boost_factor) {
  const float value = (float)idx / (float)(kGainLutN - 1u);
  const float log_boost = (float)(log2_min * (double)(1.0f - value) + log2_max * (double)value);
  return (float)exp2((double)(log_boost * boost_factor));
}

__global__ void __launch_bounds__(256) k_build_luts(float* lut) {
  const uint32_t i = blockIdx.x * 256u + threadIdx.x;
  if (i >= kLutTotal) return;
  float y;
  if (i < kLutHlgInv) y = srgb_inv_oetf_exact((float)(i - kLutSrgbInv) / (float)(kLutSrgbInvN - 1u));
  else if (i < kLutPqInv) y = hlg_inv_oetf_exact((float)(i - kLutHlgInv) / (float)(kLutHlgInvN - 1u));
  else if (i < kLutHlg) y = pq_inv_oetf_exact((float)(i - kLutPqInv) / (float)(kLutPqInvN - 1u));
  else if (i < kLutPq) y = hlg_oetf_exact((float)(i - kLutHlg) / (float)(kLutHlgN - 1u));
  else y = pq_oetf_exact((float)(i - kLutPq) / (float)(kLutPqN - 1u));
  lut[i] = y;
}
hipError_t launch_build_luts(float* lut, hipStream_t s) {
  hipLaunchKernelGGL(k_build_luts, dim3((kLutTotal + 255u) / 256u), dim3(256), 0, s, lut);
  return hipGetLastError();
}
__global__ void __launch_bounds__(256) k_build_lut_codes(float* lut) {
  const uint32_t i = blockIdx.x * 256u + threadIdx.x;
  const uint32_t t = i >> 16, k = i & 0xFFFFu;
  uint16_t* codes = reinterpret_cast<uint16_t*>(lut + (t ? kCodePq : kCodeHlg));
  codes[k] = (uint16_t)(0x3ffu & (uint32_t)(lut[(t ? kLutPq : kLutHlg) + k] * 1023.0f));
}
hipError_t launch_build_lut_codes(float* lut, hipStream_t s) {
  hipLaunchKernelGGL(k_build_lut_codes, dim3(2u * 65536u / 256u), dim3(256), 0, s, lut);
  return hipGetLastError();
}
__global__ void __launch_bounds__(256) k_build_gain_lut(float* table, double log2_min, double log2_max, float boost_factor) {
  const uint32_t i = blockIdx.x * 256u + threadIdx.x;
  if (i < kGainLutN) table[i] = gain_lut_entry(i, log2_min, log2_max, boost_factor);
}
hipError_t launch_build_gain_lut(float* table, double log2_min, double log2_max, float boost_factor, hipStream_t s) {
  hipLaunchKernelGGL(k_build_gain_lut, dim3(kGainLutN / 256u), dim3(256), 0, s, table, log2_min, log2_max, boost_factor);
  return hipGetLastError();
}


template <int TF>
__device__ __forceinline__ float hdr_inv_oetf(float e) {
  if (TF == 1) return hlg_inv_oetf_guarded(e);
  if (TF == 2) return pq_inv_oetf_guarded(e);
  return e;
}

__device__ __forceinline__ float cvt_word0(uint32_t w) {
  float r;
  asm("v_cvt_f32_u32_sdwa %0, %1 dst_sel:DWORD dst_unused:UNUSED_PAD src0_sel:WORD_0" : "=v"(r) : "v"(w));
  return r;
}
__device__ __forceinline__ float cvt_word1(uint32_t w) {
  float r;
  asm("v_cvt_f32_u32_sdwa %0, %1 dst_sel:DWORD dst_unused:UNUSED_PAD src0_sel:WORD_1" : "=v"(r) : "v"(w));
  return r;
}


constexpr int kGenWhole = 0, kGenFront = 1, kGenBack = 2;
struct GenMid { f2 r, g, b, hr, hg, hb; };
template <int TF, bool LUT, bool FILTER, bool DEFER = false, int PART = kGenWhole>
__device__ __forceinline__ uint32_t gen_pair(const GenConsts& c, const uint32_t (&hy)[2][4][2],
                                             const uint32_t (&huv)[2][2][2], const uint32_t (&y8)[2][4],
                                             const uint32_t (&u8)[2][2], const uint32_t (&v8)[2][2],
                                             uint8_t (&out)[2], float (&gain)[2], const float* s_srgb, const float* s_hdr,
                                             GenMid* mid = nullptr) {
  f2 r, g, b, hr, hg, hb;
  if (PART == kGenBack) {
    r = mid->r; g = mid->g; b = mid->b; hr = mid->hr; hg = mid->hg; hb = mid->hb;
  } else {
  f2 sy = splat(0.0f), su = splat(0.0f), sv = splat(0.0f);
  f2 hsy = splat(0.0f), hsu = splat(0.0f), hsv = splat(0.0f);
#pragma unroll
  for (int r = 0; r < 2; ++r) {
    f2 uf[2], vf[2], huf[2], hvf[2];
#pragma unroll
    for (int k = 0; k < 2; ++k) {
      const f2 ub = (f2){(float)((u8[0][r] >> (8 * k)) & 0xffu), (float)((u8[1][r] >> (8 * k)) & 0xffu)};
      const f2 vb = (f2){(float)((v8[0][r] >> (8 * k)) & 0xffu), (float)((v8[1][r] >> (8 * k)) & 0xffu)};
      uf[k] = pk_fma(ub, splat(k255), splat(-128.0f * k255));
      vf[k] = pk_fma(vb, splat(k255), splat(-128.0f * k255));
      const uint32_t m0 = huv[0][r][k] & 0xFFC0FFC0u, m1 = huv[1][r][k] & 0xFFC0FFC0u;
      const f2 hu = (f2){cvt_word0(m0), cvt_word0(m1)};
      const f2 hv = (f2){cvt_word1(m0), cvt_word1(m1)};
      huf[k] = pk_fma(hu, splat(k896 * 0.015625f), splat(-64.0f * k896)) - splat(0.5f);
      hvf[k] = pk_fma(hv, splat(k896 * 0.015625f), splat(-64.0f * k896)) - splat(0.5f);
    }
#pragma unroll
    for (int d = 0; d < 2; ++d) {
      const int dy = 2 * r + d;
#pragma unroll
      for (int dx = 0; dx < 4; ++dx) {
        const f2 yb = (f2){(float)((y8[0][dy] >> (8 * dx)) & 0xffu), (float)((y8[1][dy] >> (8 * dx)) & 0xffu)};
        sy += yb * splat(k255);
        su += uf[dx >> 1];
        sv += vf[dx >> 1];
        const uint32_t w0 = hy[0][dy][dx >> 1] & 0xFFC0FFC0u, w1 = hy[1][dy][dx >> 1] & 0xFFC0FFC0u;
        const f2 hb = (dx & 1) ? (f2){cvt_word1(w0), cvt_word1(w1)} : (f2){cvt_word0(w0), cvt_word0(w1)};
        hsy += pk_fma(hb, splat(k876 * 0.015625f), splat(-64.0f * k876));
        hsu += huf[dx >> 1];
        hsv += hvf[dx >> 1];
      }
    }
  }
  sy *= splat(0.0625f); su *= splat(0.0625f); sv *= splat(0.0625f);
  hsy *= splat(0.0625f); hsu *= splat(0.0625f); hsv *= splat(0.0625f);

  r = pk_add_sat(sy, splat(c.sdr_cr) * sv);
  g = pk_add_sat(sy - splat(c.sdr_gcb) * su, -(splat(c.sdr_gcr) * sv));
  b = pk_add_sat(sy, splat(c.sdr_cb) * su);
  hr = pk_add_sat(hsy, splat(c.hdr_cr) * hsv);
  hg = pk_add_sat(hsy - splat(c.hdr_gcb) * hsu, -(splat(c.hdr_gcr) * hsv));
  hb = pk_add_sat(hsy, splat(c.hdr_cb) * hsu);
  }
  if (PART != kGenBack && mid != nullptr) { mid->r = r; mid->g = g; mid->b = b; mid->hr = hr; mid->hg = hg; mid->hb = hb; }
  if (PART == kGenFront) return 0u;

  if (FILTER && !LUT) {
    const f2 fr = (f2){srgb_inv_oetf_fast(r.x), srgb_inv_oetf_fast(r.y)};
    const f2 fg = (f2){srgb_inv_oetf_fast(g.x), srgb_inv_oetf_fast(g.y)};
    const f2 fb = (f2){srgb_inv_oetf_fast(b.x), srgb_inv_oetf_fast(b.y)};
    const f2 fs = (splat(c.lum_r) * fr + splat(c.lum_g) * fg + splat(c.lum_b) * fb) * splat(203.0f);
    f2 qr = hr, qg = hg, qb = hb;
    if (TF == 1) {
      qr = (f2){hlg_inv_oetf_fast(hr.x), hlg_inv_oetf_fast(hr.y)};
      qg = (f2){hlg_inv_oetf_fast(hg.x), hlg_inv_oetf_fast(hg.y)};
      qb = (f2){hlg_inv_oetf_fast(hb.x), hlg_inv_oetf_fast(hb.y)};
    } else if (TF == 2) {
      qr = (f2){pq_inv_oetf_fast(hr.x), pq_inv_oetf_fast(hr.y)};
      qg = (f2){pq_inv_oetf_fast(hg.x), pq_inv_oetf_fast(hg.y)};
      qb = (f2){pq_inv_oetf_fast(hb.x), pq_inv_oetf_fast(hb.y)};
    }
    if (!c.gm_identity) {
      const f2 t0 = splat(c.gm[0]) * qr + splat(c.gm[1]) * qg + splat(c.gm[2]) * qb;
      const f2 t1 = splat(c.gm[3]) * qr + splat(c.gm[4]) * qg + splat(c.gm[5]) * qb;
      const f2 t2 = splat(c.gm[6]) * qr + splat(c.gm[7]) * qg + splat(c.gm[8]) * qb;
      qr = t0; qg = t1; qb = t2;
    }
    const f2 fh = (splat(c.lum_r) * qr + splat(c.lum_g) * qg + splat(c.lum_b) * qb) * splat(c.hdr_white_nits);
    uint32_t fbyte[2], fexact = 0u, doubt = 0u;
    float fgain[2];
#pragma unroll
    for (int k = 0; k < 2; ++k) {
      const float ys = k ? fs.y : fs.x, yh = k ? fh.y : fh.x;
      const float gf = (ys > 0.0f) ? yh * __builtin_amdgcn_rcpf(ys) : 1.0f;
      const float gc = __builtin_amdgcn_fmed3f(gf, c.min_boost, c.max_boost);
      const float v = (__builtin_amdgcn_logf(gc) - c.log2_min) * c.flt_scale;
      const float fl = __builtin_floorf(v), fr2 = v - fl;
      const bool lo = gf < c.flt_lo, hi = gf > c.flt_hi;
      const bool mid = (fr2 >= c.flt_delta) && (fr2 <= 1.0f - c.flt_delta);
      const bool sane = !(ys > 0.0f && ys < 1e-10f) && !(yh != 0.0f && __builtin_fabsf(yh) < 1e-10f);
      if (!((lo || hi || mid) && sane)) doubt |= 1u << k;
      fbyte[k] = lo ? c.enc_byte_min : hi ? c.enc_byte_max : (uint32_t)fl;
      fgain[k] = gf;
      if (!(ys > 0.0f)) fexact |= 1u << k;
    }
    if (DEFER || __builtin_amdgcn_ballot_w64(doubt != 0u) == 0ull) {
      out[0] = (uint8_t)fbyte[0]; out[1] = (uint8_t)fbyte[1];
      gain[0] = fgain[0]; gain[1] = fgain[1];
      return fexact | (doubt << 2);
    }
  }
  constexpr int kLockstep = 6;
  if (LUT) {
    r = (f2){s_srgb[lut_index_unit(r.x, kLutSrgbInvN)], s_srgb[lut_index_unit(r.y, kLutSrgbInvN)]};
    g = (f2){s_srgb[lut_index_unit(g.x, kLutSrgbInvN)], s_srgb[lut_index_unit(g.y, kLutSrgbInvN)]};
    b = (f2){s_srgb[lut_index_unit(b.x, kLutSrgbInvN)], s_srgb[lut_index_unit(b.y, kLutSrgbInvN)]};
  } else {
    float ch[6] = {r.x, r.y, g.x, g.y, b.x, b.y};
#pragma unroll
    for (int i = 0; i < 6; i += kLockstep) {
      float part[kLockstep];
#pragma unroll
      for (int j = 0; j < kLockstep; ++j) part[j] = ch[i + j];
      srgb_inv_oetf_guarded_n<kLockstep>(part);
#pragma unroll
      for (int j = 0; j < kLockstep; ++j) ch[i + j] = part[j];
    }
    r = (f2){ch[0], ch[1]}; g = (f2){ch[2], ch[3]}; b = (f2){ch[4], ch[5]};
  }
  const f2 sdr_nits = (splat(c.lum_r) * r + splat(c.lum_g) * g + splat(c.lum_b) * b) * splat(203.0f);

  if (TF != 0 && LUT) {
    hr = (f2){s_hdr[lut_index_unit(hr.x, kLutHlgInvN)], s_hdr[lut_index_unit(hr.y, kLutHlgInvN)]};
    hg = (f2){s_hdr[lut_index_unit(hg.x, kLutHlgInvN)], s_hdr[lut_index_unit(hg.y, kLutHlgInvN)]};
    hb = (f2){s_hdr[lut_index_unit(hb.x, kLutHlgInvN)], s_hdr[lut_index_unit(hb.y, kLutHlgInvN)]};
  } else if (TF != 0) {
    float ch[6] = {hr.x, hr.y, hg.x, hg.y, hb.x, hb.y};
#pragma unroll
    for (int i = 0; i < 6; i += kLockstep) {
      float part[kLockstep];
#pragma unroll
      for (int j = 0; j < kLockstep; ++j) part[j] = ch[i + j];
      if (TF == 1) hlg_inv_oetf_guarded_n<kLockstep>(part);
      else pq_inv_oetf_guarded_n<kLockstep>(part);
#pragma unroll
      for (int j = 0; j < kLockstep; ++j) ch[i + j] = part[j];
    }
    hr = (f2){ch[0], ch[1]}; hg = (f2){ch[2], ch[3]}; hb = (f2){ch[4], ch[5]};
  }
  if (!c.gm_identity) {
    const f2 t0 = splat(c.gm[0]) * hr + splat(c.gm[1]) * hg + splat(c.gm[2]) * hb;
    const f2 t1 = splat(c.gm[3]) * hr + splat(c.gm[4]) * hg + splat(c.gm[5]) * hb;
    const f2 t2 = splat(c.gm[6]) * hr + splat(c.gm[7]) * hg + splat(c.gm[8]) * hb;
    hr = t0; hg = t1; hb = t2;
  }
  const f2 hdr_nits = (splat(c.lum_r) * hr + splat(c.lum_g) * hg + splat(c.lum_b) * hb) * splat(c.hdr_white_nits);

  gain[0] = raw_gain(sdr_nits.x, hdr_nits.x);
  gain[1] = raw_gain(sdr_nits.y, hdr_nits.y);
#pragma unroll
  for (int k = 0; k < 2; ++k)
    out[k] = encode_gain_guarded(gain[k], c.min_boost, c.max_boost, c.log2_min, c.log2_max, c.enc_scale, c.enc_byte_min,
                                 c.enc_byte_max);
  return 3u;
}

typedef uint32_t u32x4 __attribute__((ext_vector_type(4)));
typedef uint32_t u32x2 __attribute__((ext_vector_type(2)));
__device__ __forceinline__ uint4 ld_stream(const uint4* p) {
  const u32x4 v = __builtin_nontemporal_load(reinterpret_cast<const u32x4*>(p));
  return make_uint4(v.x, v.y, v.z, v.w);
}
__device__ __forceinline__ uint2 ld_stream(const uint2* p) {
  const u32x2 v = __builtin_nontemporal_load(reinterpret_cast<const u32x2*>(p));
  return make_uint2(v.x, v.y);
}
__device__ __forceinline__ uint32_t ld_stream(const uint32_t* p) {
  return __builtin_nontemporal_load(p);
}
__device__ __forceinline__ void st_stream(uint4* p, uint4 v) {
  __builtin_nontemporal_store((u32x4){v.x, v.y, v.z, v.w}, reinterpret_cast<u32x4*>(p));
}
__device__ __forceinline__ void st_stream(uint2* p, uint2 v) {
  __builtin_nontemporal_store((u32x2){v.x, v.y}, reinterpret_cast<u32x2*>(p));
}
__device__ __forceinline__ uint32_t ld8(const uint8_t* p) { return *p; }
__device__ __forceinline__ uint32_t ld16(const uint16_t* p) { return *p; }

constexpr int kGenBlock = 256, kGenTiles = 4;

template <bool ALIGNED>
__device__ __forceinline__ void load_pair(const GenConsts& c, const GenImage& im, const uint8_t* im_v, uint32_t my, uint32_t pr,
                                          bool two, uint32_t (&hy)[2][4][2], uint32_t (&huv)[2][2][2], uint32_t (&y8)[2][4],
                                          uint32_t (&u8)[2][2], uint32_t (&v8)[2][2]) {
  const uint32_t mx = pr * 2u;
  if (ALIGNED) {
    const uint32_t hoff = 4u * my * im.hy_stride + 8u * pr, yoff = 4u * my * im.y_stride + 8u * pr;
#pragma unroll
    for (int r = 0; r < 4; ++r) {
      const uint4 q = ld_stream(reinterpret_cast<const uint4*>(im.hy + (hoff + r * im.hy_stride)));
      hy[0][r][0] = q.x; hy[0][r][1] = q.y; hy[1][r][0] = q.z; hy[1][r][1] = q.w;
      const uint2 p = ld_stream(reinterpret_cast<const uint2*>(im.y + (yoff + r * im.y_stride)));
      y8[0][r] = p.x; y8[1][r] = p.y;
    }
    const uint32_t huvoff = 2u * my * im.huv_stride + 8u * pr, coff = 2u * my * im.c_stride + 4u * pr;
#pragma unroll
    for (int r = 0; r < 2; ++r) {
      const uint4 q = ld_stream(reinterpret_cast<const uint4*>(im.huv + (huvoff + r * im.huv_stride)));
      huv[0][r][0] = q.x; huv[0][r][1] = q.y; huv[1][r][0] = q.z; huv[1][r][1] = q.w;
      const uint32_t uu = ld_stream(reinterpret_cast<const uint32_t*>(im.u + (coff + r * im.c_stride)));
      const uint32_t vv = ld_stream(reinterpret_cast<const uint32_t*>(im_v + (coff + r * im.c_stride)));
      u8[0][r] = uu & 0xffffu; u8[1][r] = uu >> 16;
      v8[0][r] = vv & 0xffffu; v8[1][r] = vv >> 16;
    }
  } else {
#pragma unroll
    for (int k = 0; k < 2; ++k) {
      const bool on = (k == 0) || two;
      const uint32_t x0 = 4u * (mx + k);
#pragma unroll
      for (int r = 0; r < 4; ++r) {
        const uint16_t* hrow = im.hy + (size_t)(4u * my + r) * im.hy_stride + x0;
        const uint8_t* yrow = im.y + (size_t)(4u * my + r) * im.y_stride + x0;
        hy[k][r][0] = on ? (ld16(hrow) | (ld16(hrow + 1) << 16)) : 0u;
        hy[k][r][1] = on ? (ld16(hrow + 2) | (ld16(hrow + 3) << 16)) : 0u;
        y8[k][r] = on ? (ld8(yrow) | (ld8(yrow + 1) << 8) | (ld8(yrow + 2) << 16) | (ld8(yrow + 3) << 24)) : 0u;
      }
#pragma unroll
      for (int r = 0; r < 2; ++r) {
        const uint16_t* crow = im.huv + (size_t)(2u * my + r) * im.huv_stride + x0;
        const uint8_t* urow = im.u + (size_t)(2u * my + r) * im.c_stride + (x0 >> 1);
        const uint8_t* vrow = im_v + (size_t)(2u * my + r) * im.c_stride + (x0 >> 1);
        huv[k][r][0] = on ? (ld16(crow) | (ld16(crow + 1) << 16)) : 0u;
        huv[k][r][1] = on ? (ld16(crow + 2) | (ld16(crow + 3) << 16)) : 0u;
        u8[k][r] = on ? (ld8(urow) | (ld8(urow + 1) << 8)) : 0u;
        v8[k][r] = on ? (ld8(vrow) | (ld8(vrow + 1) << 8)) : 0u;
      }
    }
  }
}

template <int CTRL, int ROWS>
__device__ __forceinline__ float dpp_move(float v) {
  return __int_as_float(__builtin_amdgcn_update_dpp(__float_as_int(v), __float_as_int(v), CTRL, ROWS, 0xF, false));
}
__device__ __forceinline__ void wave_minmax(float& vmin, float& vmax) {
  vmin = fminf(vmin, dpp_move<0xB1, 0xF>(vmin));  vmax = fmaxf(vmax, dpp_move<0xB1, 0xF>(vmax));
  vmin = fminf(vmin, dpp_move<0x4E, 0xF>(vmin));  vmax = fmaxf(vmax, dpp_move<0x4E, 0xF>(vmax));
  vmin = fminf(vmin, dpp_move<0x141, 0xF>(vmin)); vmax = fmaxf(vmax, dpp_move<0x141, 0xF>(vmax));
  vmin = fminf(vmin, dpp_move<0x140, 0xF>(vmin)); vmax = fmaxf(vmax, dpp_move<0x140, 0xF>(vmax));
  vmin = fminf(vmin, dpp_move<0x142, 0xA>(vmin)); vmax = fmaxf(vmax, dpp_move<0x142, 0xA>(vmax));
  vmin = fminf(vmin, dpp_move<0x143, 0xC>(vmin)); vmax = fmaxf(vmax, dpp_move<0x143, 0xC>(vmax));
  vmin = __int_as_float(__builtin_amdgcn_readlane(__float_as_int(vmin), 63));
  vmax = __int_as_float(__builtin_amdgcn_readlane(__float_as_int(vmax), 63));
}
__device__ __forceinline__ void publish_minmax(float gmin, float gmax, uint32_t* keys) {
  if ((threadIdx.x & 63u) == 0u && gmin <= gmax) {
    const uint32_t kmin = ~float_to_key(gmin), kmax = float_to_key(gmax);
    if (__hip_atomic_load(&keys[0], __ATOMIC_RELAXED, __HIP_MEMORY_SCOPE_AGENT) < kmin) atomicMax(&keys[0], kmin);
    if (__hip_atomic_load(&keys[1], __ATOMIC_RELAXED, __HIP_MEMORY_SCOPE_AGENT) < kmax) atomicMax(&keys[1], kmax);
  }
}

template <int TF, bool ALIGNED, bool LUT>
__device__ __forceinline__ void exact_pair(const GenConsts& c, const GenImage& im, const uint8_t* im_v, uint32_t my,
                                           uint32_t pr, bool two, const float* s_srgb, const float* s_hdr, uint8_t (&o)[2], float (&gn)[2]) {
  uint32_t hy[2][4][2], huv[2][2][2], y8[2][4], u8[2][2], v8[2][2];
  load_pair<ALIGNED>(c, im, im_v, my, pr, two, hy, huv, y8, u8, v8);
  gen_pair<TF, LUT, false>(c, hy, huv, y8, u8, v8, o, gn, s_srgb, s_hdr);
}


template <int TF, bool ALIGNED, bool LUT, bool FILTER, int TILES, bool DEFER, int BLOCK = kGenBlock>
__global__ void __launch_bounds__(BLOCK, 1) k_generate(const GenConsts c, const GenBatch b) {
  __shared__ float s_srgb[LUT ? kLutSrgbInvN : 1];
  __shared__ float s_hdr[(LUT && TF != 0) ? kLutHlgInvN : 1];
  __shared__ float s_kept[(FILTER && DEFER) ? TILES * 2 * BLOCK : 1];
  if (LUT) {
    for (uint32_t i = threadIdx.x; i < kLutSrgbInvN / 4u; i += BLOCK)
      reinterpret_cast<float4*>(s_srgb)[i] = reinterpret_cast<const float4*>(c.lut + kLutSrgbInv)[i];
    if (TF != 0) {
      const float4* src = reinterpret_cast<const float4*>(c.lut + (TF == 1 ? kLutHlgInv : kLutPqInv));
      for (uint32_t i = threadIdx.x; i < kLutHlgInvN / 4u; i += BLOCK) reinterpret_cast<float4*>(s_hdr)[i] = src[i];
    }
    __syncthreads();
  }
  const uint32_t img_i = blockIdx.x, blk = blockIdx.y;
  const GenImage& im = b.img[img_i];
  const uint8_t* im_v = im.u + (size_t)im.c_stride * (c.height / 2u);
  const uint32_t pairs_per_row = (c.map_w + 1u) >> 1;
  const uint32_t total = pairs_per_row * c.map_h;
  const bool stats = c.stat_keys != nullptr;
  float emin = __builtin_inff(), emax = -__builtin_inff();
  float amin = __builtin_inff(), amax = -__builtin_inff();
  uint32_t kept_exact = 0u, kept_valid = 0u, kept_doubt = 0u;
  uint32_t n_saved = 0u;
  uint32_t* wslot = (FILTER && DEFER && c.stat_slots != 0u)
                        ? c.stat_ws + (size_t)kStatWords * blockIdx.x + kStatHdr + (blockIdx.y * (uint32_t)(BLOCK / 64) + (threadIdx.x >> 6)) * kStatSlotWords
                        : nullptr;

#pragma unroll 1
  for (uint32_t t = 0; t < (uint32_t)TILES; ++t) {
    const uint32_t idx = (blk * (uint32_t)TILES + t) * (uint32_t)BLOCK + threadIdx.x;
    if (idx >= total) break;
    const uint32_t my = idx / pairs_per_row;
    const uint32_t pr = idx - my * pairs_per_row;
    const uint32_t mx = pr * 2u;
    const bool two = ALIGNED || (mx + 1u < c.map_w);

    uint32_t hy[2][4][2], huv[2][2][2], y8[2][4], u8[2][2], v8[2][2];
    load_pair<ALIGNED>(c, im, im_v, my, pr, two, hy, huv, y8, u8, v8);

    uint8_t o[2];
    float gn[2];
    GenMid mid;
    const uint32_t ex = gen_pair<TF, LUT, FILTER, DEFER>(c, hy, huv, y8, u8, v8, o, gn, s_srgb, s_hdr, (FILTER && DEFER) ? &mid : nullptr);
    const uint8_t o0 = o[0], o1 = o[1];
    if (FILTER && DEFER) {
      uint32_t dm = (ex >> 2) & (two ? 3u : 1u);
      if (c.stat_slots != 0u) {
        const unsigned long long dmask = __builtin_amdgcn_ballot_w64(dm != 0u);
        if (dmask != 0ull) {
          const uint32_t pos = n_saved + (uint32_t)__builtin_popcountll(dmask & ((1ull << (threadIdx.x & 63u)) - 1ull));
          n_saved += (uint32_t)__builtin_popcountll(dmask);
          if (dm != 0u && pos < kStatSlotSaved) {
            float4* e = reinterpret_cast<float4*>(wslot + 16u + pos * 16u);
            e[0] = make_float4(__uint_as_float((idx << 3) | dm), mid.r.x, mid.r.y, mid.g.x);
            e[1] = make_float4(mid.g.y, mid.b.x, mid.b.y, mid.hr.x);
            e[2] = make_float4(mid.hr.y, mid.hg.x, mid.hg.y, mid.hb.x);
            e[3] = make_float4(mid.hb.y, 0.0f, 0.0f, 0.0f);
            dm = 0u;
          }
        }
      }
      kept_doubt |= dm << (2u * t);
      if (stats) {
        s_kept[(2u * t) * BLOCK + threadIdx.x] = gn[0];
        s_kept[(2u * t + 1u) * BLOCK + threadIdx.x] = gn[1];
        const uint32_t valid = (two ? 3u : 1u) & ~((ex >> 2) & 3u);
        kept_exact |= (ex & 3u) << (2u * t);
        kept_valid |= valid << (2u * t);
        if (valid & 1u) { amin = fminf(amin, gn[0]); amax = fmaxf(amax, gn[0]); }
        if (valid & 2u) { amin = fminf(amin, gn[1]); amax = fmaxf(amax, gn[1]); }
        if (ex & valid & 1u) { emin = fminf(emin, gn[0]); emax = fmaxf(emax, gn[0]); }
        if (ex & valid & 2u) { emin = fminf(emin, gn[1]); emax = fmaxf(emax, gn[1]); }
      }
    } else {
      emin = fminf(emin, gn[0]); emax = fmaxf(emax, gn[0]);
      if (two) { emin = fminf(emin, gn[1]); emax = fmaxf(emax, gn[1]); }
    }
    uint8_t* mp = im.map + (size_t)my * c.map_w + mx;
    if (ALIGNED) {
      *reinterpret_cast<uint16_t*>(mp) = (uint16_t)(o0 | ((uint32_t)o1 << 8));
    } else {
      mp[0] = o0;
      if (two) mp[1] = o1;
    }
  }
  if (FILTER && !DEFER) return;
  if (!FILTER && !stats) return;
  uint32_t* keys = stats ? c.stat_keys + (size_t)c.stat_stride * img_i : nullptr;

  if (FILTER) {
    uint32_t* ws = c.stat_ws + (size_t)kStatWords * img_i;
    uint32_t cand = 0u;
    if (stats) {
      wave_minmax(amin, amax);
      float wmin = emin, wmax = emax;
      wave_minmax(wmin, wmax);
      const float e = c.flt_gain_rel;
      uint32_t* est = c.stat_spread != 0u ? ws + kStatEst + 2u * (blk % kStatLists) : ws;
      uint32_t e0 = __hip_atomic_load(&est[0], __ATOMIC_RELAXED, __HIP_MEMORY_SCOPE_AGENT);
      uint32_t e1 = __hip_atomic_load(&est[1], __ATOMIC_RELAXED, __HIP_MEMORY_SCOPE_AGENT);
      const uint32_t k0 = __hip_atomic_load(&keys[0], __ATOMIC_RELAXED, __HIP_MEMORY_SCOPE_AGENT);
      const uint32_t k1 = __hip_atomic_load(&keys[1], __ATOMIC_RELAXED, __HIP_MEMORY_SCOPE_AGENT);
      if (amin <= amax) {
        const uint32_t m0 = ~float_to_key(amin), m1 = float_to_key(amax);
        if ((threadIdx.x & 63u) == 0u) {
          if (e0 < m0) atomicMax(&est[0], m0);
          if (e1 < m1) atomicMax(&est[1], m1);
        }
        e0 = e0 < m0 ? m0 : e0; e1 = e1 < m1 ? m1 : e1;
      }
      float min_hi = fminf(k1 != 0u ? key_to_float(~k0) : __builtin_inff(), wmin);
      float max_lo = fmaxf(k1 != 0u ? key_to_float(k1) : -__builtin_inff(), wmax);
      if (e1 != 0u) {
        const float pmin = key_to_float(~e0), pmax = key_to_float(e1);
        min_hi = fminf(min_hi, pmin + e * __builtin_fabsf(pmin));
        max_lo = fmaxf(max_lo, pmax - e * __builtin_fabsf(pmax));
      }
#pragma unroll
      for (uint32_t t = 0; t < (uint32_t)TILES; ++t)
#pragma unroll
        for (uint32_t k = 0; k < 2u; ++k) {
          const uint32_t bit = 1u << (2u * t + k);
          if ((kept_valid & bit) && !(kept_exact & bit)) {
            const float a = s_kept[(2u * t + k) * BLOCK + threadIdx.x], slack = e * __builtin_fabsf(a);
            if ((a - slack <= min_hi) || (a + slack >= max_lo)) cand |= 1u << t;
          }
        }
    }
    unsigned long long mask[TILES];
    uint32_t total = 0u;
#pragma unroll
    for (uint32_t t = 0; t < (uint32_t)TILES; ++t) {
      mask[t] = __builtin_amdgcn_ballot_w64((((kept_doubt >> (2u * t)) & 3u) | ((cand >> t) & 1u)) != 0u);
      total += (uint32_t)__builtin_popcountll(mask[t]);
    }
    if (total != 0u || c.stat_slots != 0u) {
      const uint32_t lane = threadIdx.x & 63u, list = blk % kStatLists;
      uint32_t base = 0u, cap = kStatCap;
      uint32_t* lw = ws + kStatHdr + list * kStatCap;
      if (c.stat_slots != 0u) {
        lw = wslot;
        const bool over = total > kStatSlotPlain;
        const uint32_t ns = n_saved < kStatSlotSaved ? n_saved : kStatSlotSaved;
        if (lane == 0u) {
          ws[kStatSlotCnt + blk * (uint32_t)(BLOCK / 64) + (threadIdx.x >> 6)] = over ? 0u : (total | (ns << 8));
          if (over) __hip_atomic_store(&ws[6], 1u, __ATOMIC_RELAXED, __HIP_MEMORY_SCOPE_AGENT);
        }
        ++lw;
        cap = over ? 0u : kStatSlotPlain;
      } else {
        if (lane == 0u) base = atomicAdd(&ws[8u + list], total);
        base = (uint32_t)__builtin_amdgcn_readfirstlane((int)base);
      }
#pragma unroll
      for (uint32_t t = 0; t < (uint32_t)TILES; ++t) {
        const uint32_t flags = ((kept_doubt >> (2u * t)) & 3u) | (((cand >> t) & 1u) << 2);
        const uint32_t pos = base + (uint32_t)__builtin_popcountll(mask[t] & ((1ull << lane) - 1ull));
        if (flags != 0u && pos < cap) lw[pos] = (((blk * (uint32_t)TILES + t) * (uint32_t)BLOCK + threadIdx.x) << 3) | flags;
        base += (uint32_t)__builtin_popcountll(mask[t]);
      }
    }
    if (!stats) return;
  }
  wave_minmax(emin, emax);
  publish_minmax(emin, emax, keys);
}

__global__ void k_stats_finalize(uint32_t* keys, int n) {
  const int i = blockIdx.x * blockDim.x + threadIdx.x;
  if (i >= n) return;
  const uint32_t k0 = keys[2 * i], k1 = keys[2 * i + 1];
  float mn = __builtin_inff(), mx = -__builtin_inff();
  if (k1 != 0u) { mn = key_to_float(~k0); mx = key_to_float(k1); }
  keys[2 * i] = __float_as_uint(mn);
  keys[2 * i + 1] = __float_as_uint(mx);
}

constexpr uint32_t kResolveSlices = 16;
static_assert(kStatLists == 64u, "k_generate_resolve reads the list counts with one wave");
template <int TF, bool ALIGNED>
__global__ void __launch_bounds__(256) k_generate_resolve(const GenConsts c, const GenBatch b) {
  const uint32_t img_i = blockIdx.x;
  const GenImage& im = b.img[img_i];
  const uint8_t* im_v = im.u + (size_t)im.c_stride * (c.height / 2u);
  uint32_t* ws = c.stat_ws + (size_t)kStatWords * img_i;
  const uint32_t pairs_per_row = (c.map_w + 1u) >> 1, total = pairs_per_row * c.map_h;
  const bool stats = c.stat_out != nullptr;
  float emin = __builtin_inff(), emax = -__builtin_inff();
  __shared__ uint32_t s_first[kStatSlotWaves + 1u];
  __shared__ uint8_t s_ns[kStatSlotWaves];
  __shared__ uint32_t s_sweep;
  const bool slots = c.stat_slots != 0u;
  if (slots) {
    static_assert(kStatSlotWaves == 4u * 256u, "four waves' counts per thread");
    __shared__ uint32_t s_part[4];
    uint32_t n4[4];
    const uint4 cw4 = *reinterpret_cast<const uint4*>(ws + kStatSlotCnt + 4u * threadIdx.x);
    const uint32_t cws[4] = {cw4.x, cw4.y, cw4.z, cw4.w};
#pragma unroll
    for (uint32_t j = 0; j < 4u; ++j) {
      const uint32_t w = 4u * threadIdx.x + j;
      const uint32_t cw = w < c.stat_slots ? cws[j] : 0u;
      s_ns[w] = (uint8_t)(cw >> 8);
      n4[j] = (cw & 0xFFu) + (cw >> 8);
    }
    const uint32_t over = __hip_atomic_load(&ws[6], __ATOMIC_RELAXED, __HIP_MEMORY_SCOPE_AGENT);
    const uint32_t mine = n4[0] + n4[1] + n4[2] + n4[3];
    const uint32_t before = block_exclusive_sum<256>(mine, s_part);
    s_first[4u * threadIdx.x] = before;
    s_first[4u * threadIdx.x + 1u] = before + n4[0];
    s_first[4u * threadIdx.x + 2u] = before + n4[0] + n4[1];
    s_first[4u * threadIdx.x + 3u] = before + n4[0] + n4[1] + n4[2];
    if (threadIdx.x == 255u) { s_first[kStatSlotWaves] = before + mine; s_sweep = over; }
  } else if (threadIdx.x < 64u) {
    const uint32_t cnt = ws[8u + threadIdx.x];
    const bool over = __builtin_amdgcn_ballot_w64(cnt > kStatCap) != 0ull;
    uint32_t inc = min(cnt, kStatCap);
#pragma unroll
    for (int off = 1; off < 64; off <<= 1) {
      const uint32_t v = (uint32_t)__shfl_up((int)inc, off, 64);
      if ((int)threadIdx.x >= off) inc += v;
    }
    s_first[threadIdx.x + 1u] = inc;
    if (threadIdx.x == 0) { s_first[0] = 0u; s_sweep = over ? 1u : 0u; }
  }
  __syncthreads();
  const bool sweep = s_sweep != 0u;
  const uint32_t nl = slots ? kStatSlotWaves : kStatLists;
  const uint32_t n = sweep ? total : s_first[nl];
#pragma unroll 1
  for (uint32_t g = blockIdx.y * 256u + threadIdx.x; g < n; g += kResolveSlices * 256u) {
    uint32_t entry = (g << 3) | 7u;
    GenMid mid;
    bool have = false;
    if (!sweep) {
      uint32_t l = 0u;
      for (uint32_t s2 = nl / 2u; s2 != 0u; s2 >>= 1) if (s_first[l + s2] <= g) l += s2;
      const uint32_t k = g - s_first[l];
      if (!slots) {
        entry = ws[kStatHdr + l * kStatCap + k];
      } else if (k >= (uint32_t)s_ns[l]) {
        entry = ws[kStatHdr + l * kStatSlotWords + 1u + (k - (uint32_t)s_ns[l])];
      } else {
        const uint4* e = reinterpret_cast<const uint4*>(ws + kStatHdr + l * kStatSlotWords + 16u + k * 16u);
        const uint4 e0 = e[0], e1 = e[1], e2 = e[2], e3 = e[3];
        entry = e0.x;
        mid.r = (f2){__uint_as_float(e0.y), __uint_as_float(e0.z)};
        mid.g = (f2){__uint_as_float(e0.w), __uint_as_float(e1.x)};
        mid.b = (f2){__uint_as_float(e1.y), __uint_as_float(e1.z)};
        mid.hr = (f2){__uint_as_float(e1.w), __uint_as_float(e2.x)};
        mid.hg = (f2){__uint_as_float(e2.y), __uint_as_float(e2.z)};
        mid.hb = (f2){__uint_as_float(e2.w), __uint_as_float(e3.x)};
        have = true;
      }
    }
    const uint32_t idx = entry >> 3;
    const uint32_t my = idx / pairs_per_row, pr = idx - my * pairs_per_row;
    const bool two = ALIGNED || (pr * 2u + 1u < c.map_w);
    uint8_t o[2];
    float gn[2];
    uint32_t hy[2][4][2], huv[2][2][2], y8[2][4], u8[2][2], v8[2][2];
    if (!have) {
      load_pair<ALIGNED>(c, im, im_v, my, pr, two, hy, huv, y8, u8, v8);
      gen_pair<TF, false, false, false, kGenFront>(c, hy, huv, y8, u8, v8, o, gn, nullptr, nullptr, &mid);
    }
    gen_pair<TF, false, false, false, kGenBack>(c, hy, huv, y8, u8, v8, o, gn, nullptr, nullptr, &mid);
    uint8_t* mp = im.map + (size_t)my * c.map_w + 2u * pr;
    if (entry & 1u) mp[0] = o[0];
    if ((entry & 2u) && two) mp[1] = o[1];
    if ((entry & 5u) != 0u) { emin = fminf(emin, gn[0]); emax = fmaxf(emax, gn[0]); }
    if ((entry & 6u) != 0u && two) { emin = fminf(emin, gn[1]); emax = fmaxf(emax, gn[1]); }
  }
  if (stats) {
    wave_minmax(emin, emax);
    publish_minmax(emin, emax, ws + 4);
  }
  __shared__ uint32_t s_last;
  asm volatile("s_waitcnt vmcnt(0)" ::: "memory");
  __syncthreads();
  if (threadIdx.x == 0) s_last = atomicAdd(&ws[3], 1u);
  __syncthreads();
  if (s_last == kResolveSlices - 1u && threadIdx.x == 0) {
    if (stats) {
      const uint32_t k0 = __hip_atomic_load(&ws[4], __ATOMIC_RELAXED, __HIP_MEMORY_SCOPE_AGENT);
      const uint32_t k1 = __hip_atomic_load(&ws[5], __ATOMIC_RELAXED, __HIP_MEMORY_SCOPE_AGENT);
      float mn = __builtin_inff(), mx = -__builtin_inff();
      if (k1 != 0u) { mn = key_to_float(~k0); mx = key_to_float(k1); }
      c.stat_out[2u * img_i] = mn;
      c.stat_out[2u * img_i + 1u] = mx;
    }
  }
  __syncthreads();
  static_assert(kStatSlotCnt <= 256u, "one header word per thread");
  if (s_last == kResolveSlices - 1u && threadIdx.x < kStatSlotCnt)
    __hip_atomic_store(&ws[threadIdx.x], 0u, __ATOMIC_RELAXED, __HIP_MEMORY_SCOPE_AGENT);
}
template <int TF>
static hipError_t launch_stats_resolve_tf(const GenConsts& c, const GenBatch& b, int n, bool aligned, hipStream_t s) {
  if (aligned) hipLaunchKernelGGL((k_generate_resolve<TF, true>), dim3((unsigned)n, kResolveSlices), dim3(256), 0, s, c, b);
  else hipLaunchKernelGGL((k_generate_resolve<TF, false>), dim3((unsigned)n, kResolveSlices), dim3(256), 0, s, c, b);
  return hipGetLastError();
}
hipError_t launch_stats_resolve(const GenConsts& c, const GenBatch& b, int n, int hdr_tf, bool aligned, hipStream_t s) {
  if (n <= 0 || c.stat_ws == nullptr) return hipSuccess;
  switch (hdr_tf) {
    case 0: return launch_stats_resolve_tf<0>(c, b, n, aligned, s);
    case 1: return launch_stats_resolve_tf<1>(c, b, n, aligned, s);
    case 2: return launch_stats_resolve_tf<2>(c, b, n, aligned, s);
    default: return hipErrorInvalidValue;
  }
}

bool generate_is_small(const GenConsts& c, int n) {
  const uint32_t total = ((c.map_w + 1u) >> 1) * c.map_h;
  const uint32_t span = (uint32_t)kGenBlock * (uint32_t)kGenTiles;
  return (uint64_t)((total + span - 1u) / span) * (uint64_t)n < 1024u;
}

uint32_t generate_slot_waves(const GenConsts& c, int n) {
  const uint32_t total = ((c.map_w + 1u) >> 1) * c.map_h;
  const uint32_t per = (uint32_t)kGenBlock * (generate_is_small(c, n) ? 1u : (uint32_t)kGenTiles);
  const uint64_t waves = (uint64_t)((total + per - 1u) / per) * (uint64_t)(kGenBlock / 64);
  return waves <= kStatSlotWaves ? (uint32_t)waves : 0u;
}

bool generate_resolve_pays(const GenConsts& c, int n) {
  const uint32_t total = ((c.map_w + 1u) >> 1) * c.map_h;
  const uint32_t span = (uint32_t)kGenBlock * (uint32_t)kGenTiles;
  return (uint64_t)((total + span - 1u) / span) * (uint64_t)n >= 128u;
}

template <int TF, bool ALIGNED, bool LUT, bool FILTER>
static hipError_t launch_generate_t(const GenConsts& c, const GenBatch& b, int n, hipStream_t s) {
  const uint32_t total = ((c.map_w + 1u) >> 1) * c.map_h;
  if (total == 0 || n == 0) return hipSuccess;
  const bool small = generate_is_small(c, n);
  const unsigned b4 = (total + (uint32_t)kGenBlock * (uint32_t)kGenTiles - 1u) / ((uint32_t)kGenBlock * (uint32_t)kGenTiles);
  const unsigned b1 = (total + kGenBlock - 1u) / kGenBlock;
  const dim3 g4 = dim3((unsigned)n, b4, 1);
  const dim3 g1 = dim3((unsigned)n, b1, 1);
  if (FILTER) {
    if (c.stat_ws != nullptr) {
      if (small) hipLaunchKernelGGL((k_generate<TF, ALIGNED, LUT, FILTER, 1, true>), g1, dim3(kGenBlock, 1, 1), 0, s, c, b);
      else hipLaunchKernelGGL((k_generate<TF, ALIGNED, LUT, FILTER, kGenTiles, true>), g4, dim3(kGenBlock, 1, 1), 0, s, c, b);
    } else {
      if (c.stat_keys != nullptr) return hipErrorInvalidValue;
      const unsigned h1 = (total + 127u) / 128u;
      if ((uint64_t)h1 * (uint64_t)n >= 2000u) {
        const dim3 gh = dim3((unsigned)n, h1, 1);
        hipLaunchKernelGGL((k_generate<TF, ALIGNED, LUT, FILTER, 1, false, 128>), gh, dim3(128, 1, 1), 0, s, c, b);
      } else {
        hipLaunchKernelGGL((k_generate<TF, ALIGNED, LUT, FILTER, 1, false>), g1, dim3(kGenBlock, 1, 1), 0, s, c, b);
      }
    }
  } else if (small) {
    hipLaunchKernelGGL((k_generate<TF, ALIGNED, LUT, FILTER, 1, false>), g1, dim3(kGenBlock, 1, 1), 0, s, c, b);
  } else {
    hipLaunchKernelGGL((k_generate<TF, ALIGNED, LUT, FILTER, kGenTiles, false>), g4, dim3(kGenBlock, 1, 1), 0, s, c, b);
  }
  return hipGetLastError();
}

template <int TF>
static hipError_t launch_generate_tf(const GenConsts& c, const GenBatch& b, int n, bool aligned, bool lut, bool filter,
                                     hipStream_t s) {
  if (lut) return aligned ? launch_generate_t<TF, true, true, false>(c, b, n, s) : launch_generate_t<TF, false, true, false>(c, b, n, s);
  if (filter && aligned) return launch_generate_t<TF, true, false, true>(c, b, n, s);
  return aligned ? launch_generate_t<TF, true, false, false>(c, b, n, s) : launch_generate_t<TF, false, false, false>(c, b, n, s);
}
hipError_t launch_generate(const GenConsts& c, const GenBatch& b, int n, int hdr_tf, bool aligned, bool lut,
                           bool filter, hipStream_t s) {
  if (lut && c.lut == nullptr) return hipErrorInvalidValue;
  switch (hdr_tf) {
    case 0: return launch_generate_tf<0>(c, b, n, aligned, lut, filter, s);
    case 1: return launch_generate_tf<1>(c, b, n, aligned, lut, filter, s);
    case 2: return launch_generate_tf<2>(c, b, n, aligned, lut, filter, s);
    default: return hipErrorInvalidValue;
  }
}

hipError_t launch_stats_init(uint32_t* keys, int n, hipStream_t s) {
  return hipMemsetAsync(keys, 0, sizeof(uint32_t) * 2 * (size_t)n, s);
}
hipError_t launch_stats_finalize(uint32_t* keys, int n, hipStream_t s) {
  if (n == 0) return hipSuccess;
  hipLaunchKernelGGL(k_stats_finalize, dim3((n + 63) / 64), dim3(64), 0, s, keys, n);
  return hipGetLastError();
}



template <bool EXACT>
__device__ __forceinline__ F3 recover_hdr(const AppConsts& c, float yf, float crv, float gcbu,
                                          float gcrv, float cbu, float gain) {
  float r = clamp01(yf + crv);
  float g = clamp01(yf - gcbu - gcrv);
  float b = clamp01(yf + cbu);
  const float log_boost = (float)(c.log2_min_d * (double)(1.0f - gain) + c.log2_max_d * (double)gain);
  F3 o;
  if (EXACT) {
    float ch[3] = {r, g, b};
    srgb_inv_oetf_guarded_n<3>(ch);
    r = ch[0]; g = ch[1]; b = ch[2];
    const float factor = exp2_to_float_guarded(log_boost * c.display_boost / c.max_boost);
    o.x = (r * factor) / c.display_boost;
    o.y = (g * factor) / c.display_boost;
    o.z = (b * factor) / c.display_boost;
  } else {
    r = srgb_inv_oetf_fast(r); g = srgb_inv_oetf_fast(g); b = srgb_inv_oetf_fast(b);
    const float factor = __builtin_amdgcn_exp2f((log_boost * c.display_boost) * c.inv_max_boost);
    o.x = (r * factor) * c.inv_display_boost;
    o.y = (g * factor) * c.inv_display_boost;
    o.z = (b * factor) * c.inv_display_boost;
  }
  return o;
}

template <int FMT, bool EXACT>
__device__ __forceinline__ F3 hdr_oetf(F3 e) {
  if (FMT == 3) {
    if (EXACT) { float ch[3] = {e.x, e.y, e.z}; hlg_oetf_guarded_n<3>(ch); e.x = ch[0]; e.y = ch[1]; e.z = ch[2]; }
    else { e.x = hlg_oetf_fast(e.x); e.y = hlg_oetf_fast(e.y); e.z = hlg_oetf_fast(e.z); }
  } else if (FMT == 2) {
    if (EXACT) { float ch[3] = {e.x, e.y, e.z}; pq_oetf_guarded_n<3>(ch); e.x = ch[0]; e.y = ch[1]; e.z = ch[2]; }
    else { e.x = pq_oetf_est(e.x); e.y = pq_oetf_est(e.y); e.z = pq_oetf_est(e.z); }
  }
  return e;
}

__device__ __forceinline__ float map_to_float(uint32_t v) { return (float)v / 255.0f; }
__device__ __forceinline__ float map_to_float_fast(uint32_t v) { return div_const((float)v, 255.0f, 1.0f / 255.0f); }

__device__ __forceinline__ f2 log2_2(f2 v) { return (f2){__builtin_amdgcn_logf(v.x), __builtin_amdgcn_logf(v.y)}; }
__device__ __forceinline__ f2 exp2_2(f2 v) { return (f2){__builtin_amdgcn_exp2f(v.x), __builtin_amdgcn_exp2f(v.y)}; }
__device__ __forceinline__ f2 sqrt_2(f2 v) { return (f2){__builtin_amdgcn_sqrtf(v.x), __builtin_amdgcn_sqrtf(v.y)}; }
__device__ __forceinline__ f2 rcp_2(f2 v) { return (f2){__builtin_amdgcn_rcpf(v.x), __builtin_amdgcn_rcpf(v.y)}; }
__device__ __forceinline__ f2 sel_le(f2 x, float thr, f2 a, f2 b) {
  return (f2){x.x <= thr ? a.x : b.x, x.y <= thr ? a.y : b.y};
}


__device__ __forceinline__ f2 srgb_eotf2(f2 e) {
  constexpr float kThr = 0.04045f;
  const f2 a = pk_mul_sat(e, splat(1.0f / kThr));
  const f2 lin = pk_fma(a, splat(kThr / 12.92f), splat(-(kThr / 12.92f)));
  const f2 d = pk_add_sat(e, splat(-kThr));
  const f2 x = pk_fma(d, splat(1.0f / 1.055f), splat((kThr + 0.055f) / 1.055f));
  const f2 t = exp2_2(log2_2(x) * splat(0.4f));
  return pk_fma(x * x, t, lin);
}

__device__ __forceinline__ uint32_t tab_offset(float x) {
  typedef __fp16 h2 __attribute__((ext_vector_type(2)));
  const h2 q = __builtin_amdgcn_cvt_pkrtz(x, 0.0f);
  return __builtin_bit_cast(uint32_t, q) & 0x7FF8u;
}
__device__ __forceinline__ uint32_t pow_offset(float x) {
  uint32_t off;
  asm("v_and_b32_sdwa %0, %1, %2 dst_sel:DWORD dst_unused:UNUSED_PAD src0_sel:DWORD src1_sel:WORD_1" : "=v"(off) : "v"(0x0FF8u), "v"(x));
  return off;
}
__device__ __forceinline__ void pow_pair(f2 x, const char* lut, float2& a, float2& b) {
  a = *reinterpret_cast<const float2*>(lut + pow_offset(x.x));
  b = *reinterpret_cast<const float2*>(lut + pow_offset(x.y));
}
template <uint32_t BASE>
__device__ __forceinline__ void tab_pair(f2 x, const char* lut, float2& a, float2& b) {
  typedef __fp16 h2 __attribute__((ext_vector_type(2)));
  const h2 q = __builtin_amdgcn_cvt_pkrtz(x.x, x.y);
  const uint32_t d = __builtin_bit_cast(uint32_t, q);
  uint32_t hi_off;
  asm("v_and_b32_sdwa %0, %1, %2 dst_sel:DWORD dst_unused:UNUSED_PAD src0_sel:DWORD src1_sel:WORD_1" : "=v"(hi_off) : "v"(0x7FF8u), "v"(d));
  a = *reinterpret_cast<const float2*>(lut + BASE + (d & 0x7FF8u));
  b = *reinterpret_cast<const float2*>(lut + BASE + hi_off);
}
template <uint32_t BASE>
__device__ __forceinline__ f2 tab_eval2(f2 x, const char* lut) {
  float2 a, b;
  tab_pair<BASE>(x, lut, a, b);
  f2 o;
  asm("v_fma_f32 %0, %1, %2, %3" : "=v"(o.x) : "v"(a.y), "v"(x.x), "v"(a.x));
  asm("v_fma_f32 %0, %1, %2, %3" : "=v"(o.y) : "v"(b.y), "v"(x.y), "v"(b.x));
  return o;
}
__device__ __forceinline__ uint32_t s2_address(float s, uint32_t slot8) {
  return __builtin_amdgcn_perm(__float_as_uint(s), slot8, 0x0C0C0600u);
}
__device__ __forceinline__ f2 code_eval2(f2 s, uint32_t slot8, const char* lut) {
  const float2 a = *reinterpret_cast<const float2*>(lut + s2_address(s.x, slot8));
  const float2 b = *reinterpret_cast<const float2*>(lut + s2_address(s.y, slot8));
  f2 o;
  asm("v_fma_f32 %0, %1, %2, %3" : "=v"(o.x) : "v"(a.y), "v"(s.x), "v"(a.x));
  asm("v_fma_f32 %0, %1, %2, %3" : "=v"(o.y) : "v"(b.y), "v"(s.y), "v"(b.x));
  return o;
}

template <int FMT, bool MASK> struct ApplyTab {
  static constexpr bool kOetf = !MASK && (FMT == 2 || FMT == 3);
  static constexpr uint32_t kS1Bytes = kOetf ? kTabS1PowBytes : kTabS1Bytes;
  static constexpr uint32_t kS2Base = kS1Bytes;
  static constexpr uint32_t kS2Bytes = kOetf ? kTabS2LdsBytes : 0u;
  static constexpr uint32_t kBytes = kS1Bytes + kS2Bytes;
  static constexpr uint32_t kS1Float = !kOetf ? kTabS1Lin : FMT == 3 ? kTabS1Hlg : kTabS1Pq;
  static constexpr uint32_t kS2Float = FMT == 3 ? kTabS2Hlg : kTabS2Pq;
};

template <int FMT>
__device__ __forceinline__ f2 oetf2_scaled(f2 e) {
  if (FMT == 3) {
    const f2 lo = sqrt_2(e * splat(3.0f * 1023.0f * 1023.0f));
    const f2 hi = pk_fma(log2_2(pk_fma(e, splat(12.0f), splat(-UHDR_HLG_B))),
                         splat(UHDR_HLG_A * 0.693147180559945f * 1023.0f), splat(UHDR_HLG_C * 1023.0f));
    return sel_le(e, 1.0f / 12.0f, lo, hi);
  } else if (FMT == 2) {
    const f2 p = exp2_2(log2_2(e) * splat(UHDR_PQ_M1));
    const f2 q = pk_fma(p, splat(UHDR_PQ_C2), splat(UHDR_PQ_C1)) * rcp_2(pk_fma(p, splat(UHDR_PQ_C3), splat(1.0f)));
    return exp2_2(pk_fma(log2_2(q), splat(UHDR_PQ_M2), splat(9.99859042974533f)));
  } else if (FMT == 4) {
    return e * splat(1023.0f);
  }
  return e;
}

struct PairOut { f2 r, g, b; };

template <bool MASK>
__device__ __forceinline__ uint32_t pack10_scaled(float r, float g, float b) {
  uint32_t ri = (uint32_t)r, gi = (uint32_t)g, bi = (uint32_t)b;
  if (MASK) { ri &= 0x3ffu; gi &= 0x3ffu; bi &= 0x3ffu; }
  uint32_t t;
  asm("v_lshl_or_b32 %0, %1, 10, %2" : "=v"(t) : "v"(gi), "v"(ri));
  asm("v_lshl_or_b32 %0, %1, 20, %2" : "=v"(t) : "v"(bi), "v"(t));
  return t | 0xC0000000u;
}
__device__ __forceinline__ uint32_t pack10_bits(float r, float g, float b) {
  uint32_t t;
  asm("v_lshl_or_b32 %0, %1, 10, %2" : "=v"(t) : "v"(__float_as_uint(g)), "v"(__float_as_uint(r)));
  asm("v_lshl_or_b32 %0, %1, 20, %2" : "=v"(t) : "v"(__float_as_uint(b)), "v"(t));
  return t;
}

template <int K>
__device__ __forceinline__ float cvt_byte(uint32_t w) { return (float)((w >> (8 * K)) & 0xffu); }

struct PairF { f2 c[3]; f2 factor; float2 e[6]; };
struct PairM { f2 s[3]; float2 e[6]; };
struct ChromaRow { f2 crv, ngs, cbu; };
__device__ __forceinline__ ChromaRow chroma_row(uint32_t uu, uint32_t vv) {
  constexpr float kCrS = kP3Cr * k255, kCbS = kP3Cb * k255, kGCbS = kP3GCb * k255, kGCrS = kP3GCr * k255;
  const f2 uf = (f2){cvt_byte<0>(uu), cvt_byte<1>(uu)};
  const f2 vf = (f2){cvt_byte<0>(vv), cvt_byte<1>(vv)};
  ChromaRow o;
  o.crv = pk_fma(vf, splat(kCrS), splat(-128.0f * kCrS));
  o.cbu = pk_fma(uf, splat(kCbS), splat(-128.0f * kCbS));
  o.ngs = pk_fma(uf, splat(-kGCbS), pk_fma(vf, splat(-kGCrS), splat(128.0f * kGCbS + 128.0f * kGCrS)));
  return o;
}
template <int FMT>
__device__ __forceinline__ void apply_cell_piped(const AppConsts& c, void* dst, uint32_t cx, uint32_t cy,
                                                 const uint32_t (&yrow)[4], const uint32_t (&uu)[2], const uint32_t (&vv)[2],
                                                 float m1, float m2, float m3, float m4, uint32_t slot8, const char* lut) {
  typedef ApplyTab<FMT, false> T;
  ChromaRow cr = chroma_row(uu[0], vv[0]);
  const float a255 = c.fast.A255;
  f2 d23 = (f2){m2 - m1, m3 - m1}, d4b = (f2){m4 - m1, __builtin_fmaf(m1, a255, c.fast.B)};
  asm("" : "+v"(d23), "+v"(d4b));
  PairF pf[2];
  PairM pm[2];
  uint32_t px[4];
#pragma unroll
  for (int k = 0; k < 10; ++k) {
    if (k < 8) {
      const int oy = k >> 1, pr = k & 1;
      const f2 w1 = (f2){c.fast.wD[oy][pr][0][0], c.fast.wD[oy][pr][0][1]}, w2 = (f2){c.fast.wD[oy][pr][1][0], c.fast.wD[oy][pr][1][1]};
      const f2 w3 = (f2){c.fast.wD[oy][pr][2][0], c.fast.wD[oy][pr][2][1]};
      if (k == 4) cr = chroma_row(uu[1], vv[1]);
      PairF& f = pf[k & 1];
      const f2 E = pk_fma(bc_lo(d4b), w3, pk_fma(bc_hi(d23), w2, pk_fma(bc_lo(d23), w1, bc_hi(d4b))));
      const f2 yraw = pr ? (f2){cvt_byte<2>(yrow[oy]), cvt_byte<3>(yrow[oy])} : (f2){cvt_byte<0>(yrow[oy]), cvt_byte<1>(yrow[oy])};
      if (pr) {
        f.c[0] = pk_fma_sat_bc<1>(yraw, splat(k255), cr.crv); f.c[1] = pk_fma_sat_bc<1>(yraw, splat(k255), cr.ngs);
        f.c[2] = pk_fma_sat_bc<1>(yraw, splat(k255), cr.cbu);
      } else {
        f.c[0] = pk_fma_sat_bc<0>(yraw, splat(k255), cr.crv); f.c[1] = pk_fma_sat_bc<0>(yraw, splat(k255), cr.ngs);
        f.c[2] = pk_fma_sat_bc<0>(yraw, splat(k255), cr.cbu);
      }
      f.factor = exp2_2(E);
#pragma unroll
      for (int ch = 0; ch < 3; ++ch) pow_pair(f.c[ch], lut, f.e[2 * ch], f.e[2 * ch + 1]);
    }
    __builtin_amdgcn_sched_barrier(0);
    if (k >= 1 && k <= 8) {
      PairF& f = pf[(k - 1) & 1];
      PairM& m = pm[(k - 1) & 1];
#pragma unroll
      for (int ch = 0; ch < 3; ++ch) {
        f2 t;
        asm("v_fma_f32 %0, %1, %2, %3" : "=v"(t.x) : "v"(f.e[2 * ch].y), "v"(f.c[ch].x), "v"(f.e[2 * ch].x));
        asm("v_fma_f32 %0, %1, %2, %3" : "=v"(t.y) : "v"(f.e[2 * ch + 1].y), "v"(f.c[ch].y), "v"(f.e[2 * ch + 1].x));
        m.s[ch] = pk_fma(t, f.factor, splat(2.0f));
      }
#pragma unroll
      for (int ch = 0; ch < 3; ++ch) {
        m.e[2 * ch] = *reinterpret_cast<const float2*>(lut + T::kS2Base + s2_address(m.s[ch].x, slot8));
        m.e[2 * ch + 1] = *reinterpret_cast<const float2*>(lut + T::kS2Base + s2_address(m.s[ch].y, slot8));
      }
    }
    __builtin_amdgcn_sched_barrier(0);
    if (k >= 2) {
      const int q = k - 2, oy = q >> 1, pr = q & 1;
      PairM& m = pm[q & 1];
      float o[6];
#pragma unroll
      for (int ch = 0; ch < 3; ++ch) {
        asm("v_fma_f32 %0, %1, %2, %3" : "=v"(o[2 * ch]) : "v"(m.e[2 * ch].y), "v"(m.s[ch].x), "v"(m.e[2 * ch].x));
        asm("v_fma_f32 %0, %1, %2, %3" : "=v"(o[2 * ch + 1]) : "v"(m.e[2 * ch + 1].y), "v"(m.s[ch].y), "v"(m.e[2 * ch + 1].x));
      }
      px[2 * pr] = pack10_bits(o[0], o[2], o[4]);
      px[2 * pr + 1] = pack10_bits(o[1], o[3], o[5]);
      if (pr) {
        const uint32_t off = ((4u * cy + oy) * c.width + 4u * cx) * 4u;
        st_stream(reinterpret_cast<uint4*>(static_cast<char*>(dst) + off), make_uint4(px[0], px[1], px[2], px[3]));
      }
    }
    __builtin_amdgcn_sched_barrier(0);
  }
}

constexpr uint32_t kXchSecond = 72;
constexpr uint32_t kXchPerWave = 136;
template <int FMT, bool MASK>
__device__ __forceinline__ void apply_cell_piped1(const AppConsts& c, const AppImage& im, uint32_t cx, uint32_t cy,
// ... 1457 lines not shown
```

Baseline: 541,300.

## Fold deferred exact-resolve pass into generate kernel with block-local LDS lists

Removes the separate k_generate_resolve launch. Each generate block now collects its doubtful and candidate pixel pairs in a shared-memory list and re-evaluates them in place after a block barrier. Min/max is merged per block, and the last block writes the output stats and clears the workspace. The intent is to drop a second kernel launch, the global per-wave slot and list storage, and the global scan over it. The cost is an extra block barrier and serial tail work inside every generate block, plus a full-tile sweep when a block's list overflows. A lighter lockstep setting is also used for PQ in the back half.

```diff
diff --git a/libultrahdr_dev_amd/csrc/uhdr_capi.hip b/libultrahdr_dev_amd/csrc/uhdr_capi.hip
--- a/libultrahdr_dev_amd/csrc/uhdr_capi.hip
+++ b/libultrahdr_dev_amd/csrc/uhdr_capi.hip
@@ -256,7 +256,6 @@
   c.stat_ws = nullptr;
   c.stat_out = nullptr;
   c.stat_spread = 0u;
-  c.stat_slots = 0u;
   c.lut = nullptr;
   c.bias4096 = 4096.0f;
   const double kRel = hdr_tf == UHDR_HIP_TF_PQ ? 1.0e-5 : 4.0e-6, kLogAbs = 5.0e-7;
@@ -2760,12 +2759,12 @@
     }
     bool filter = generate_mode == UHDR_HIP_GENERATE_EXACT && c.flt_delta < 0.25f && c.min_boost >= 0.25f && c.max_boost <= 64.0f;
     const bool small = generate_is_small(c, m);
-    const bool pair = keys != nullptr ? generate_resolve_pays(c, m) : !small;
-    if (keys != nullptr && !pair) filter = false;
-    const bool resolve = filter && aligned && !lut && pair;
+    const bool defer_ok = keys != nullptr ? generate_filter_pays(c, m) : !small;
+    if (keys != nullptr && !defer_ok) filter = false;
+    const bool defer = filter && aligned && !lut && defer_ok;
     std::unique_lock<std::mutex> pair_lk(g_pair_mu, std::defer_lock);
-    if (resolve) pair_lk.lock();
-    if (resolve) {
+    if (defer) {
+      pair_lk.lock();
       uint32_t* w = nullptr;
       const int wrc = stat_workspace(st, s, &w);
       if (wrc != UHDR_HIP_NO_ERROR) return wrc;
@@ -2774,13 +2773,11 @@
       c.stat_stride = kStatWords;
       c.stat_out = keys ? content_minmax + 2 * i : nullptr;
       c.stat_spread = (m <= 16 && (uint64_t)((c.map_w + 1u) >> 1) * c.map_h >= 512u * 64u) ? 1u : 0u;
-      c.stat_slots = generate_slot_waves(c, m);
     } else if (keys != nullptr) {
       HIP_TRY(launch_stats_init(keys + 2 * i, m, s));
     }
     HIP_TRY(launch_generate(c, b, m, hdr_tf, aligned, lut, filter, s));
-    if (resolve) HIP_TRY(launch_stats_resolve(c, b, m, hdr_tf, aligned, s));
-    else if (keys != nullptr) HIP_TRY(launch_stats_finalize(keys + 2 * i, m, s));
+    if (!defer && keys != nullptr) HIP_TRY(launch_stats_finalize(keys + 2 * i, m, s));
     i += m;
   }
   return UHDR_HIP_NO_ERROR;
diff --git a/libultrahdr_dev_amd/csrc/uhdr_kernels.h b/libultrahdr_dev_amd/csrc/uhdr_kernels.h
--- a/libultrahdr_dev_amd/csrc/uhdr_kernels.h
+++ b/libultrahdr_dev_amd/csrc/uhdr_kernels.h
@@ -4,11 +4,7 @@
 
 namespace uhdr {
 
-constexpr uint32_t kStatSlotWaves = 1024, kStatSlotPlain = 15, kStatSlotSaved = 4, kStatSlotWords = 16 + 16 * kStatSlotSaved;
-constexpr uint32_t kStatLists = 64, kStatCap = 252, kStatEst = 8 + kStatLists, kStatSlotCnt = kStatEst + 2 * kStatLists,
-                   kStatHdr = kStatSlotCnt + kStatSlotWaves,
-                   kStatWords = kStatHdr + (kStatLists * kStatCap > kStatSlotWaves * kStatSlotWords ? kStatLists * kStatCap : kStatSlotWaves * kStatSlotWords);
-static_assert(kStatHdr % 4u == 0u && kStatSlotWords % 4u == 0u && kStatWords % 4u == 0u, "saved entries are read and written as 16-byte pieces");
+constexpr uint32_t kStatSpread = 64, kStatEst = 8, kStatTicket = kStatEst + 2 * kStatSpread, kStatWords = kStatTicket + kStatSpread;
 constexpr int kMaxChunk = 64;
 
 constexpr uint32_t kLutSrgbInvN = 1024, kLutHlgInvN = 4096, kLutPqInvN = 4096, kLutHlgN = 65536, kLutPqN = 65536;
@@ -43,7 +39,6 @@
   float flt_scale, flt_delta, flt_lo, flt_hi;
   float flt_gain_rel;
   uint32_t stat_spread;
-  uint32_t stat_slots;
 };
 struct EvalConsts {
   float min_boost, max_boost, log2_min, log2_max;
@@ -147,10 +142,8 @@
 hipError_t launch_generate(const GenConsts& c, const GenBatch& b, int n, int hdr_tf, bool aligned, bool lut,
                            bool filter, hipStream_t s);
 bool generate_is_small(const GenConsts& c, int n);
-bool generate_resolve_pays(const GenConsts& c, int n);
-uint32_t generate_slot_waves(const GenConsts& c, int n);
+bool generate_filter_pays(const GenConsts& c, int n);
 hipError_t launch_stats_init(uint32_t* keys, int n, hipStream_t s);
-hipError_t launch_stats_resolve(const GenConsts& c, const GenBatch& b, int n, int hdr_tf, bool aligned, hipStream_t s);
 constexpr size_t kStatWsBytes = sizeof(uint32_t) * kStatWords * (size_t)kMaxChunk;
 hipError_t launch_stats_finalize(uint32_t* keys, int n, hipStream_t s);
 hipError_t launch_apply(const AppConsts& c, const AppBatch& b, int n, int fmt, int mode,
diff --git a/libultrahdr_dev_amd/csrc/uhdr_kernels.hip b/libultrahdr_dev_amd/csrc/uhdr_kernels.hip
--- a/libultrahdr_dev_amd/csrc/uhdr_kernels.hip
+++ b/libultrahdr_dev_amd/csrc/uhdr_kernels.hip
@@ -148,7 +148,7 @@
 
 constexpr int kGenWhole = 0, kGenFront = 1, kGenBack = 2;
 struct GenMid { f2 r, g, b, hr, hg, hb; };
-template <int TF, bool LUT, bool FILTER, bool DEFER = false, int PART = kGenWhole>
+template <int TF, bool LUT, bool FILTER, bool DEFER = false, int PART = kGenWhole, int LOCKSTEP = 6>
 __device__ __forceinline__ uint32_t gen_pair(const GenConsts& c, const uint32_t (&hy)[2][4][2],
                                              const uint32_t (&huv)[2][2][2], const uint32_t (&y8)[2][4],
                                              const uint32_t (&u8)[2][2], const uint32_t (&v8)[2][2],
@@ -250,7 +250,7 @@
       return fexact | (doubt << 2);
     }
   }
-  constexpr int kLockstep = 6;
+  constexpr int kLockstep = LOCKSTEP;
   if (LUT) {
     r = (f2){s_srgb[lut_index_unit(r.x, kLutSrgbInvN)], s_srgb[lut_index_unit(r.y, kLutSrgbInvN)]};
     g = (f2){s_srgb[lut_index_unit(g.x, kLutSrgbInvN)], s_srgb[lut_index_unit(g.y, kLutSrgbInvN)]};
@@ -402,20 +402,18 @@
   }
 }
 
-template <int TF, bool ALIGNED, bool LUT>
-__device__ __forceinline__ void exact_pair(const GenConsts& c, const GenImage& im, const uint8_t* im_v, uint32_t my,
-                                           uint32_t pr, bool two, const float* s_srgb, const float* s_hdr, uint8_t (&o)[2], float (&gn)[2]) {
-  uint32_t hy[2][4][2], huv[2][2][2], y8[2][4], u8[2][2], v8[2][2];
-  load_pair<ALIGNED>(c, im, im_v, my, pr, two, hy, huv, y8, u8, v8);
-  gen_pair<TF, LUT, false>(c, hy, huv, y8, u8, v8, o, gn, s_srgb, s_hdr);
-}
-
+
+constexpr uint32_t kGenListCap = 128, kGenEntryWords = 16;
 
 template <int TF, bool ALIGNED, bool LUT, bool FILTER, int TILES, bool DEFER, int BLOCK = kGenBlock>
 __global__ void __launch_bounds__(BLOCK, 1) k_generate(const GenConsts c, const GenBatch b) {
   __shared__ float s_srgb[LUT ? kLutSrgbInvN : 1];
   __shared__ float s_hdr[(LUT && TF != 0) ? kLutHlgInvN : 1];
   __shared__ float s_kept[(FILTER && DEFER) ? TILES * 2 * BLOCK : 1];
+  __shared__ __attribute__((aligned(16))) uint32_t s_list[(FILTER && DEFER) ? kGenListCap * kGenEntryWords : 4];
+  __shared__ uint32_t s_cnt;
+  __shared__ float s_mm[2 * (BLOCK / 64)];
+  static_assert(!(FILTER && DEFER) || (!LUT && ALIGNED), "the deferred form is the aligned, table-free kernel");
   if (LUT) {
     for (uint32_t i = threadIdx.x; i < kLutSrgbInvN / 4u; i += BLOCK)
       reinterpret_cast<float4*>(s_srgb)[i] = reinterpret_cast<const float4*>(c.lut + kLutSrgbInv)[i];
@@ -423,6 +421,10 @@
       const float4* src = reinterpret_cast<const float4*>(c.lut + (TF == 1 ? kLutHlgInv : kLutPqInv));
       for (uint32_t i = threadIdx.x; i < kLutHlgInvN / 4u; i += BLOCK) reinterpret_cast<float4*>(s_hdr)[i] = src[i];
     }
+    __syncthreads();
+  }
+  if (FILTER && DEFER) {
+    if (threadIdx.x == 0) s_cnt = 0u;
     __syncthreads();
   }
   const uint32_t img_i = blockIdx.x, blk = blockIdx.y;
@@ -433,11 +435,8 @@
   const bool stats = c.stat_keys != nullptr;
   float emin = __builtin_inff(), emax = -__builtin_inff();
   float amin = __builtin_inff(), amax = -__builtin_inff();
-  uint32_t kept_exact = 0u, kept_valid = 0u, kept_doubt = 0u;
-  uint32_t n_saved = 0u;
-  uint32_t* wslot = (FILTER && DEFER && c.stat_slots != 0u)
-                        ? c.stat_ws + (size_t)kStatWords * blockIdx.x + kStatHdr + (blockIdx.y * (uint32_t)(BLOCK / 64) + (threadIdx.x >> 6)) * kStatSlotWords
-                        : nullptr;
+  uint32_t kept_exact = 0u, kept_valid = 0u;
+  uint32_t seen0 = 0u, seen1 = 0u;
 
 #pragma unroll 1
   for (uint32_t t = 0; t < (uint32_t)TILES; ++t) {
@@ -457,23 +456,21 @@
     const uint32_t ex = gen_pair<TF, LUT, FILTER, DEFER>(c, hy, huv, y8, u8, v8, o, gn, s_srgb, s_hdr, (FILTER && DEFER) ? &mid : nullptr);
     const uint8_t o0 = o[0], o1 = o[1];
     if (FILTER && DEFER) {
-      uint32_t dm = (ex >> 2) & (two ? 3u : 1u);
-      if (c.stat_slots != 0u) {
-        const unsigned long long dmask = __builtin_amdgcn_ballot_w64(dm != 0u);
-        if (dmask != 0ull) {
-          const uint32_t pos = n_saved + (uint32_t)__builtin_popcountll(dmask & ((1ull << (threadIdx.x & 63u)) - 1ull));
-          n_saved += (uint32_t)__builtin_popcountll(dmask);
-          if (dm != 0u && pos < kStatSlotSaved) {
-            float4* e = reinterpret_cast<float4*>(wslot + 16u + pos * 16u);
-            e[0] = make_float4(__uint_as_float((idx << 3) | dm), mid.r.x, mid.r.y, mid.g.x);
-            e[1] = make_float4(mid.g.y, mid.b.x, mid.b.y, mid.hr.x);
-            e[2] = make_float4(mid.hr.y, mid.hg.x, mid.hg.y, mid.hb.x);
-            e[3] = make_float4(mid.hb.y, 0.0f, 0.0f, 0.0f);
-            dm = 0u;
-          }
+      const uint32_t dm = (ex >> 2) & (two ? 3u : 1u);
+      const unsigned long long dmask = __builtin_amdgcn_ballot_w64(dm != 0u);
+      if (dmask != 0ull) {
+        uint32_t base = 0u;
+        if ((threadIdx.x & 63u) == 0u) base = atomicAdd(&s_cnt, (uint32_t)__builtin_popcountll(dmask));
+        base = (uint32_t)__builtin_amdgcn_readfirstlane((int)base);
+        const uint32_t pos = base + (uint32_t)__builtin_popcountll(dmask & ((1ull << (threadIdx.x & 63u)) - 1ull));
+        if (dm != 0u && pos < kGenListCap) {
+          float4* e = reinterpret_cast<float4*>(s_list + pos * kGenEntryWords);
+          e[0] = make_float4(__uint_as_float((idx << 3) | dm), mid.r.x, mid.r.y, mid.g.x);
+          e[1] = make_float4(mid.g.y, mid.b.x, mid.b.y, mid.hr.x);
+          e[2] = make_float4(mid.hr.y, mid.hg.x, mid.hg.y, mid.hb.x);
+          e[3] = make_float4(mid.hb.y, 0.0f, 0.0f, 0.0f);
         }
       }
-      kept_doubt |= dm << (2u * t);
       if (stats) {
         s_kept[(2u * t) * BLOCK + threadIdx.x] = gn[0];
         s_kept[(2u * t + 1u) * BLOCK + threadIdx.x] = gn[1];
@@ -503,17 +500,18 @@
 
   if (FILTER) {
     uint32_t* ws = c.stat_ws + (size_t)kStatWords * img_i;
-    uint32_t cand = 0u;
     if (stats) {
+      uint32_t cand = 0u;
       wave_minmax(amin, amax);
       float wmin = emin, wmax = emax;
       wave_minmax(wmin, wmax);
       const float e = c.flt_gain_rel;
-      uint32_t* est = c.stat_spread != 0u ? ws + kStatEst + 2u * (blk % kStatLists) : ws;
+      uint32_t* est = c.stat_spread != 0u ? ws + kStatEst + 2u * (blk % kStatSpread) : ws;
       uint32_t e0 = __hip_atomic_load(&est[0], __ATOMIC_RELAXED, __HIP_MEMORY_SCOPE_AGENT);
       uint32_t e1 = __hip_atomic_load(&est[1], __ATOMIC_RELAXED, __HIP_MEMORY_SCOPE_AGENT);
       const uint32_t k0 = __hip_atomic_load(&keys[0], __ATOMIC_RELAXED, __HIP_MEMORY_SCOPE_AGENT);
       const uint32_t k1 = __hip_atomic_load(&keys[1], __ATOMIC_RELAXED, __HIP_MEMORY_SCOPE_AGENT);
+      seen0 = (uint32_t)__builtin_amdgcn_readfirstlane((int)k0); seen1 = (uint32_t)__builtin_amdgcn_readfirstlane((int)k1);
       if (amin <= amax) {
         const uint32_t m0 = ~float_to_key(amin), m1 = float_to_key(amax);
         if ((threadIdx.x & 63u) == 0u) {
@@ -539,44 +537,110 @@
             if ((a - slack <= min_hi) || (a + slack >= max_lo)) cand |= 1u << t;
           }
         }
-    }
-    unsigned long long mask[TILES];
-    uint32_t total = 0u;
-#pragma unroll
-    for (uint32_t t = 0; t < (uint32_t)TILES; ++t) {
-      mask[t] = __builtin_amdgcn_ballot_w64((((kept_doubt >> (2u * t)) & 3u) | ((cand >> t) & 1u)) != 0u);
-      total += (uint32_t)__builtin_popcountll(mask[t]);
-    }
-    if (total != 0u || c.stat_slots != 0u) {
-      const uint32_t lane = threadIdx.x & 63u, list = blk % kStatLists;
-      uint32_t base = 0u, cap = kStatCap;
-      uint32_t* lw = ws + kStatHdr + list * kStatCap;
-      if (c.stat_slots != 0u) {
-        lw = wslot;
-        const bool over = total > kStatSlotPlain;
-        const uint32_t ns = n_saved < kStatSlotSaved ? n_saved : kStatSlotSaved;
-        if (lane == 0u) {
-          ws[kStatSlotCnt + blk * (uint32_t)(BLOCK / 64) + (threadIdx.x >> 6)] = over ? 0u : (total | (ns << 8));
-          if (over) __hip_atomic_store(&ws[6], 1u, __ATOMIC_RELAXED, __HIP_MEMORY_SCOPE_AGENT);
+      unsigned long long mask[TILES];
+      uint32_t nc = 0u;
+#pragma unroll
+      for (uint32_t t = 0; t < (uint32_t)TILES; ++t) {
+        mask[t] = __builtin_amdgcn_ballot_w64(((cand >> t) & 1u) != 0u);
+        nc += (uint32_t)__builtin_popcountll(mask[t]);
+      }
+      if (nc != 0u) {
+        const uint32_t lane = threadIdx.x & 63u;
+        uint32_t base = 0u;
+        if (lane == 0u) base = atomicAdd(&s_cnt, nc);
+        base = (uint32_t)__builtin_amdgcn_readfirstlane((int)base);
+#pragma unroll
+        for (uint32_t t = 0; t < (uint32_t)TILES; ++t) {
+          const uint32_t pos = base + (uint32_t)__builtin_popcountll(mask[t] & ((1ull << lane) - 1ull));
+          if (((cand >> t) & 1u) != 0u && pos < kGenListCap)
+            s_list[pos * kGenEntryWords] = (((blk * (uint32_t)TILES + t) * (uint32_t)BLOCK + threadIdx.x) << 3) | 4u;
+          base += (uint32_t)__builtin_popcountll(mask[t]);
         }
-        ++lw;
-        cap = over ? 0u : kStatSlotPlain;
-      } else {
-        if (lane == 0u) base = atomicAdd(&ws[8u + list], total);
-        base = (uint32_t)__builtin_amdgcn_readfirstlane((int)base);
-      }
-#pragma unroll
-      for (uint32_t t = 0; t < (uint32_t)TILES; ++t) {
-        const uint32_t flags = ((kept_doubt >> (2u * t)) & 3u) | (((cand >> t) & 1u) << 2);
-        const uint32_t pos = base + (uint32_t)__builtin_popcountll(mask[t] & ((1ull << lane) - 1ull));
-        if (flags != 0u && pos < cap) lw[pos] = (((blk * (uint32_t)TILES + t) * (uint32_t)BLOCK + threadIdx.x) << 3) | flags;
-        base += (uint32_t)__builtin_popcountll(mask[t]);
-      }
+      }
+    }
+    asm volatile("s_waitcnt vmcnt(0)" ::: "memory");
+    __syncthreads();
+    const uint32_t cnt = s_cnt;
+    const bool over = cnt > kGenListCap;
+    const uint32_t n = over ? (uint32_t)TILES * (uint32_t)BLOCK : cnt;
+#pragma unroll 1
+    for (uint32_t g = threadIdx.x; g < n; g += (uint32_t)BLOCK) {
+      uint32_t entry = ((blk * (uint32_t)TILES * (uint32_t)BLOCK + g) << 3) | 7u;
+      GenMid mid;
+      bool have = false;
+      if (!over) {
+        const uint4* en = reinterpret_cast<const uint4*>(s_list + g * kGenEntryWords);
+        entry = en[0].x;
+        have = (entry & 3u) != 0u;
+        if (have) {
+          const uint4 e0 = en[0], e1 = en[1], e2 = en[2], e3 = en[3];
+          mid.r = (f2){__uint_as_float(e0.y), __uint_as_float(e0.z)};
+          mid.g = (f2){__uint_as_float(e0.w), __uint_as_float(e1.x)};
+          mid.b = (f2){__uint_as_float(e1.y), __uint_as_float(e1.z)};
+          mid.hr = (f2){__uint_as_float(e1.w), __uint_as_float(e2.x)};
+          mid.hg = (f2){__uint_as_float(e2.y), __uint_as_float(e2.z)};
+          mid.hb = (f2){__uint_as_float(e2.w), __uint_as_float(e3.x)};
+        }
+      }
+      const uint32_t idx = entry >> 3;
+      if (idx >= total) continue;
+      const uint32_t my = idx / pairs_per_row, pr = idx - my * pairs_per_row;
+      const bool two = ALIGNED || (pr * 2u + 1u < c.map_w);
+      uint8_t o[2];
+      float gn[2];
+      uint32_t hy[2][4][2], huv[2][2][2], y8[2][4], u8[2][2], v8[2][2];
+      if (!have) {
+        load_pair<ALIGNED>(c, im, im_v, my, pr, two, hy, huv, y8, u8, v8);
+        gen_pair<TF, false, false, false, kGenFront>(c, hy, huv, y8, u8, v8, o, gn, nullptr, nullptr, &mid);
+      }
+      gen_pair<TF, false, false, false, kGenBack, (TF == 2 ? 3 : 6)>(c, hy, huv, y8, u8, v8, o, gn, nullptr, nullptr, &mid);
+      uint8_t* mp = im.map + (size_t)my * c.map_w + 2u * pr;
+      if (entry & 1u) mp[0] = o[0];
+      if ((entry & 2u) && two) mp[1] = o[1];
+      if ((entry & 5u) != 0u) { emin = fminf(emin, gn[0]); emax = fmaxf(emax, gn[0]); }
+      if ((entry & 6u) != 0u && two) { emin = fminf(emin, gn[1]); emax = fmaxf(emax, gn[1]); }
     }
     if (!stats) return;
   }
   wave_minmax(emin, emax);
-  publish_minmax(emin, emax, keys);
+  if (!(FILTER && DEFER)) {
+    publish_minmax(emin, emax, keys);
+    return;
+  }
+  if ((threadIdx.x & 63u) == 0u) { s_mm[2u * (threadIdx.x >> 6)] = emin; s_mm[2u * (threadIdx.x >> 6) + 1u] = emax; }
+  __syncthreads();
+  if (threadIdx.x >= 64u) return;
+#pragma unroll
+  for (uint32_t w = 0; w < (uint32_t)(BLOCK / 64); ++w) { emin = fminf(emin, s_mm[2u * w]); emax = fmaxf(emax, s_mm[2u * w + 1u]); }
+  if (threadIdx.x == 0 && emin <= emax) {
+    const uint32_t kmin = ~float_to_key(emin), kmax = float_to_key(emax);
+    if (seen0 < kmin || seen1 < kmax) {
+      if (__hip_atomic_load(&keys[0], __ATOMIC_RELAXED, __HIP_MEMORY_SCOPE_AGENT) < kmin) atomicMax(&keys[0], kmin);
+      if (__hip_atomic_load(&keys[1], __ATOMIC_RELAXED, __HIP_MEMORY_SCOPE_AGENT) < kmax) atomicMax(&keys[1], kmax);
+    }
+  }
+  uint32_t* ws = c.stat_ws + (size_t)kStatWords * img_i;
+  asm volatile("s_waitcnt vmcnt(0)" ::: "memory");
+  uint32_t last = 0u;
+  if (threadIdx.x == 0) {
+    const uint32_t grp = blk % kStatSpread, nblk = gridDim.y;
+    if (nblk <= kStatSpread) {
+      last = atomicAdd(&ws[3], 1u) == nblk - 1u ? 1u : 0u;
+    } else if (atomicAdd(&ws[kStatTicket + grp], 1u) == (nblk - grp + kStatSpread - 1u) / kStatSpread - 1u) {
+      last = atomicAdd(&ws[3], 1u) == kStatSpread - 1u ? 1u : 0u;
+    }
+  }
+  if (__builtin_amdgcn_readfirstlane((int)last) == 0) return;
+  if (threadIdx.x == 0 && c.stat_out != nullptr) {
+    const uint32_t k0 = __hip_atomic_load(&ws[4], __ATOMIC_RELAXED, __HIP_MEMORY_SCOPE_AGENT);
+    const uint32_t k1 = __hip_atomic_load(&ws[5], __ATOMIC_RELAXED, __HIP_MEMORY_SCOPE_AGENT);
+    float mn = __builtin_inff(), mx = -__builtin_inff();
+    if (k1 != 0u) { mn = key_to_float(~k0); mx = key_to_float(k1); }
+    c.stat_out[2u * img_i] = mn;
+    c.stat_out[2u * img_i + 1u] = mx;
+  }
+  asm volatile("s_waitcnt vmcnt(0)" ::: "memory");
+  for (uint32_t i = threadIdx.x; i < kStatWords; i += 64u) __hip_atomic_store(&ws[i], 0u, __ATOMIC_RELAXED, __HIP_MEMORY_SCOPE_AGENT);
 }
 
 __global__ void k_stats_finalize(uint32_t* keys, int n) {
@@ -589,158 +653,19 @@
   keys[2 * i + 1] = __float_as_uint(mx);
 }
 
-constexpr uint32_t kResolveSlices = 16;
-static_assert(kStatLists == 64u, "k_generate_resolve reads the list counts with one wave");
-template <int TF, bool ALIGNED>
-__global__ void __launch_bounds__(256) k_generate_resolve(const GenConsts c, const GenBatch b) {
-  const uint32_t img_i = blockIdx.x;
-  const GenImage& im = b.img[img_i];
-  const uint8_t* im_v = im.u + (size_t)im.c_stride * (c.height / 2u);
-  uint32_t* ws = c.stat_ws + (size_t)kStatWords * img_i;
-  const uint32_t pairs_per_row = (c.map_w + 1u) >> 1, total = pairs_per_row * c.map_h;
-  const bool stats = c.stat_out != nullptr;
-  float emin = __builtin_inff(), emax = -__builtin_inff();
-  __shared__ uint32_t s_first[kStatSlotWaves + 1u];
-  __shared__ uint8_t s_ns[kStatSlotWaves];
-  __shared__ uint32_t s_sweep;
-  const bool slots = c.stat_slots != 0u;
-  if (slots) {
-    static_assert(kStatSlotWaves == 4u * 256u, "four waves' counts per thread");
-    __shared__ uint32_t s_part[4];
-    uint32_t n4[4];
-    const uint4 cw4 = *reinterpret_cast<const uint4*>(ws + kStatSlotCnt + 4u * threadIdx.x);
-    const uint32_t cws[4] = {cw4.x, cw4.y, cw4.z, cw4.w};
-#pragma unroll
-    for (uint32_t j = 0; j < 4u; ++j) {
-      const uint32_t w = 4u * threadIdx.x + j;
-      const uint32_t cw = w < c.stat_slots ? cws[j] : 0u;
-      s_ns[w] = (uint8_t)(cw >> 8);
-      n4[j] = (cw & 0xFFu) + (cw >> 8);
-    }
-    const uint32_t over = __hip_atomic_load(&ws[6], __ATOMIC_RELAXED, __HIP_MEMORY_SCOPE_AGENT);
-    const uint32_t mine = n4[0] + n4[1] + n4[2] + n4[3];
-    const uint32_t before = block_exclusive_sum<256>(mine, s_part);
-    s_first[4u * threadIdx.x] = before;
-    s_first[4u * threadIdx.x + 1u] = before + n4[0];
-    s_first[4u * threadIdx.x + 2u] = before + n4[0] + n4[1];
-    s_first[4u * threadIdx.x + 3u] = before + n4[0] + n4[1] + n4[2];
-    if (threadIdx.x == 255u) { s_first[kStatSlotWaves] = before + mine; s_sweep = over; }
-  } else if (threadIdx.x < 64u) {
-    const uint32_t cnt = ws[8u + threadIdx.x];
-    const bool over = __builtin_amdgcn_ballot_w64(cnt > kStatCap) != 0ull;
-    uint32_t inc = min(cnt, kStatCap);
-#pragma unroll
-    for (int off = 1; off < 64; off <<= 1) {
-      const uint32_t v = (uint32_t)__shfl_up((int)inc, off, 64);
-      if ((int)threadIdx.x >= off) inc += v;
-    }
-    s_first[threadIdx.x + 1u] = inc;
-    if (threadIdx.x == 0) { s_first[0] = 0u; s_sweep = over ? 1u : 0u; }
-  }
-  __syncthreads();
-  const bool sweep = s_sweep != 0u;
-  const uint32_t nl = slots ? kStatSlotWaves : kStatLists;
-  const uint32_t n = sweep ? total : s_first[nl];
-#pragma unroll 1
-  for (uint32_t g = blockIdx.y * 256u + threadIdx.x; g < n; g += kResolveSlices * 256u) {
-    uint32_t entry = (g << 3) | 7u;
-    GenMid mid;
-    bool have = false;
-    if (!sweep) {
-      uint32_t l = 0u;
-      for (uint32_t s2 = nl / 2u; s2 != 0u; s2 >>= 1) if (s_first[l + s2] <= g) l += s2;
-      const uint32_t k = g - s_first[l];
-      if (!slots) {
-        entry = ws[kStatHdr + l * kStatCap + k];
-      } else if (k >= (uint32_t)s_ns[l]) {
-        entry = ws[kStatHdr + l * kStatSlotWords + 1u + (k - (uint32_t)s_ns[l])];
-      } else {
-        const uint4* e = reinterpret_cast<const uint4*>(ws + kStatHdr + l * kStatSlotWords + 16u + k * 16u);
-        const uint4 e0 = e[0], e1 = e[1], e2 = e[2], e3 = e[3];
-        entry = e0.x;
-        mid.r = (f2){__uint_as_float(e0.y), __uint_as_float(e0.z)};
-        mid.g = (f2){__uint_as_float(e0.w), __uint_as_float(e1.x)};
-        mid.b = (f2){__uint_as_float(e1.y), __uint_as_float(e1.z)};
-        mid.hr = (f2){__uint_as_float(e1.w), __uint_as_float(e2.x)};
-        mid.hg = (f2){__uint_as_float(e2.y), __uint_as_float(e2.z)};
-        mid.hb = (f2){__uint_as_float(e2.w), __uint_as_float(e3.x)};
-        have = true;
-      }
-    }
-    const uint32_t idx = entry >> 3;
-    const uint32_t my = idx / pairs_per_row, pr = idx - my * pairs_per_row;
-    const bool two = ALIGNED || (pr * 2u + 1u < c.map_w);
-    uint8_t o[2];
-    float gn[2];
-    uint32_t hy[2][4][2], huv[2][2][2], y8[2][4], u8[2][2], v8[2][2];
-    if (!have) {
-      load_pair<ALIGNED>(c, im, im_v, my, pr, two, hy, huv, y8, u8, v8);
-      gen_pair<TF, false, false, false, kGenFront>(c, hy, huv, y8, u8, v8, o, gn, nullptr, nullptr, &mid);
-    }
-    gen_pair<TF, false, false, false, kGenBack>(c, hy, huv, y8, u8, v8, o, gn, nullptr, nullptr, &mid);
-    uint8_t* mp = im.map + (size_t)my * c.map_w + 2u * pr;
-    if (entry & 1u) mp[0] = o[0];
-    if ((entry & 2u) && two) mp[1] = o[1];
-    if ((entry & 5u) != 0u) { emin = fminf(emin, gn[0]); emax = fmaxf(emax, gn[0]); }
-    if ((entry & 6u) != 0u && two) { emin = fminf(emin, gn[1]); emax = fmaxf(emax, gn[1]); }
-  }
-  if (stats) {
-    wave_minmax(emin, emax);
-    publish_minmax(emin, emax, ws + 4);
-  }
-  __shared__ uint32_t s_last;
-  asm volatile("s_waitcnt vmcnt(0)" ::: "memory");
-  __syncthreads();
-  if (threadIdx.x == 0) s_last = atomicAdd(&ws[3], 1u);
-  __syncthreads();
-  if (s_last == kResolveSlices - 1u && threadIdx.x == 0) {
-    if (stats) {
-      const uint32_t k0 = __hip_atomic_load(&ws[4], __ATOMIC_RELAXED, __HIP_MEMORY_SCOPE_AGENT);
-      const uint32_t k1 = __hip_atomic_load(&ws[5], __ATOMIC_RELAXED, __HIP_MEMORY_SCOPE_AGENT);
-      float mn = __builtin_inff(), mx = -__builtin_inff();
-      if (k1 != 0u) { mn = key_to_float(~k0); mx = key_to_float(k1); }
-      c.stat_out[2u * img_i] = mn;
-      c.stat_out[2u * img_i + 1u] = mx;
-    }
-  }
-  __syncthreads();
-  static_assert(kStatSlotCnt <= 256u, "one header word per thread");
-  if (s_last == kResolveSlices - 1u && threadIdx.x < kStatSlotCnt)
-    __hip_atomic_store(&ws[threadIdx.x], 0u, __ATOMIC_RELAXED, __HIP_MEMORY_SCOPE_AGENT);
-}
-template <int TF>
-static hipError_t launch_stats_resolve_tf(const GenConsts& c, const GenBatch& b, int n, bool aligned, hipStream_t s) {
-  if (aligned) hipLaunchKernelGGL((k_generate_resolve<TF, true>), dim3((unsigned)n, kResolveSlices), dim3(256), 0, s, c, b);
-  else hipLaunchKernelGGL((k_generate_resolve<TF, false>), dim3((unsigned)n, kResolveSlices), dim3(256), 0, s, c, b);
-  return hipGetLastError();
-}
-hipError_t launch_stats_resolve(const GenConsts& c, const GenBatch& b, int n, int hdr_tf, bool aligned, hipStream_t s) {
-  if (n <= 0 || c.stat_ws == nullptr) return hipSuccess;
-  switch (hdr_tf) {
-    case 0: return launch_stats_resolve_tf<0>(c, b, n, aligned, s);
-    case 1: return launch_stats_resolve_tf<1>(c, b, n, aligned, s);
-    case 2: return launch_stats_resolve_tf<2>(c, b, n, aligned, s);
-    default: return hipErrorInvalidValue;
-  }
-}
-
 bool generate_is_small(const GenConsts& c, int n) {
   const uint32_t total = ((c.map_w + 1u) >> 1) * c.map_h;
   const uint32_t span = (uint32_t)kGenBlock * (uint32_t)kGenTiles;
   return (uint64_t)((total + span - 1u) / span) * (uint64_t)n < 1024u;
 }
 
-uint32_t generate_slot_waves(const GenConsts& c, int n) {
-  const uint32_t total = ((c.map_w + 1u) >> 1) * c.map_h;
-  const uint32_t per = (uint32_t)kGenBlock * (generate_is_small(c, n) ? 1u : (uint32_t)kGenTiles);
-  const uint64_t waves = (uint64_t)((total + per - 1u) / per) * (uint64_t)(kGenBlock / 64);
-  return waves <= kStatSlotWaves ? (uint32_t)waves : 0u;
-}
-
-bool generate_resolve_pays(const GenConsts& c, int n) {
+#ifndef UHDR_GEN_FILTER_MIN_SPANS
+#define UHDR_GEN_FILTER_MIN_SPANS 128
+#endif
+bool generate_filter_pays(const GenConsts& c, int n) {
   const uint32_t total = ((c.map_w + 1u) >> 1) * c.map_h;
   const uint32_t span = (uint32_t)kGenBlock * (uint32_t)kGenTiles;
-  return (uint64_t)((total + span - 1u) / span) * (uint64_t)n >= 128u;
+  return (uint64_t)((total + span - 1u) / span) * (uint64_t)n >= (uint64_t)(UHDR_GEN_FILTER_MIN_SPANS);
 }
 
 template <int TF, bool ALIGNED, bool LUT, bool FILTER>
```

Result: no change. 538,500 (-0.5%).
